# ElementsProject/lightning

Measured on AMD Instinct MI355X. Metric: signature verifies/sec (ECDSA+Schnorr mix), higher is better.
Workload: dtype u32 (256-bit modular integer); 1 GPU; configs[1]+configs[2]: 1000000 ECDSA (65-byte keys, 65536 distinct) + 1000000 BIP-340 Schnorr per GPU per step, 90% valid / 10% invalid, inputs resident in HBM; parallelism=shard-by-row x1, RCCL all-gather of verdicts, key_table_cache=off (tables rebuilt every call)

## Files before the change

### include/lightning_amd.h

```cpp
#ifndef LIGHTNING_AMD_H
#define LIGHTNING_AMD_H
#include <stddef.h>
#include <stdint.h>

#ifdef __cplusplus
extern "C" {
#endif

typedef struct lamd_ctx lamd_ctx;

enum {
	LAMD_OK = 0,
	LAMD_ERR_NO_DEVICE = -1,
	LAMD_ERR_HIP = -2,
	LAMD_ERR_ARG = -3,
	LAMD_ERR_NOMEM = -4,
	LAMD_ERR_STATE = -5
};

int lamd_init(lamd_ctx **ctx, int device);
void lamd_shutdown(lamd_ctx *ctx);
const char *lamd_last_error(const lamd_ctx *ctx);
const char *lamd_version(void);

// ... 117 lines not shown
	uint64_t dropped_deleted, dropped_verdict, dropped_dependency, dropped_bookkeeping;
	uint64_t out_len;
	double stage_ms[3];
} lamd_store_repair_summary;
int lamd_gossip_store_repair(lamd_ctx *ctx, const uint8_t *store, size_t len, const void *d_store, const uint8_t *uuid32, size_t cap,
			     uint64_t *rec_off, int8_t *verdict, uint64_t *new_off, uint8_t *reason, size_t *n_records, uint8_t *out,
			     void *d_out, size_t out_cap, lamd_store_summary *summary, lamd_store_repair_summary *repair);

typedef struct {
	uint64_t now;
	uint32_t future_slack;
	uint32_t prune_interval;
} lamd_store_latest_policy;
typedef struct {
	uint64_t kept;
	uint64_t dropped_deleted, dropped_verdict, dropped_dependency, dropped_bookkeeping,
		 dropped_superseded, dropped_timestamp, dropped_stale;
	uint64_t out_len;
	double stage_ms[3];
} lamd_store_latest_summary;
int lamd_gossip_store_repair_latest(lamd_ctx *ctx, const uint8_t *store, size_t len, const void *d_store, const uint8_t *uuid32,
				    const lamd_store_latest_policy *policy, size_t cap, uint64_t *rec_off, int8_t *verdict, uint64_t *new_off,
				    uint8_t *reason, size_t *n_records, uint8_t *out, void *d_out, size_t out_cap,
				    lamd_store_summary *summary, lamd_store_latest_summary *latest);

int lamd_queue_ecdsa(lamd_ctx *ctx, const uint8_t hash32[32], const uint8_t sig64[64],
		     const uint8_t *pubkey, size_t publen);
int lamd_queue_schnorr(lamd_ctx *ctx, const uint8_t msg32[32], const uint8_t xonly32[32],
		       const uint8_t sig64[64]);
int lamd_queue_ecdsa_batch(lamd_ctx *ctx, size_t n, const uint8_t *hash32, const uint8_t *sig64, const uint8_t *pubkey,
			   size_t publen, size_t pubstride);
int lamd_queue_schnorr_batch(lamd_ctx *ctx, size_t n, const uint8_t *msg32, const uint8_t *xonly32, const uint8_t *sig64);
int lamd_queue_reserve(lamd_ctx *ctx, size_t n, size_t keylen, uint8_t **hash32, uint8_t **sig64, uint8_t **key);
int lamd_queue_ecdsa_batch_inplace(lamd_ctx *ctx, size_t n, const uint8_t *hash32, const uint8_t *sig64, const uint8_t *pubkey, size_t publen);
int lamd_queue_schnorr_batch_inplace(lamd_ctx *ctx, size_t n, const uint8_t *msg32, const uint8_t *xonly32, const uint8_t *sig64);
int lamd_host_register(lamd_ctx *ctx, void *p, size_t bytes);
int lamd_host_unregister(lamd_ctx *ctx, void *p);
int lamd_device_numa_node(int device);
int lamd_flush(lamd_ctx *ctx);
int lamd_poll(lamd_ctx *ctx, uint8_t *ok, size_t cap, size_t *n);
int lamd_wait(lamd_ctx *ctx, uint8_t *ok, size_t cap, size_t *n);

typedef struct lamd_multi lamd_multi;
int lamd_multi_init(lamd_multi **m, const int *devices, int n_devices);
void lamd_multi_shutdown(lamd_multi *m);
const char *lamd_multi_last_error(const lamd_multi *m);
int lamd_multi_devices(const lamd_multi *m);
lamd_ctx *lamd_multi_ctx(lamd_multi *m, int i);
int lamd_multi_verify_ecdsa_batch(lamd_multi *m, size_t n, const uint8_t *hash32, const uint8_t *sig64, const uint8_t *pub, size_t publen,
				  size_t pubstride, size_t group_rows, uint8_t *ok);
int lamd_multi_verify_schnorr_batch(lamd_multi *m, size_t n, const uint8_t *msg32, const uint8_t *xonly32, const uint8_t *sig64, size_t group_rows,
				    uint8_t *ok);
int lamd_multi_sigcheck_gossip_batch(lamd_multi *m, size_t n, const uint8_t *msgs, const uint64_t *off, const uint8_t *node_ids33, int8_t *verdict);
int lamd_shard_bounds(size_t n_groups, const uint32_t *group_rows, int n_shards, size_t *bounds_groups, size_t *bounds_rows);



typedef struct {
	int device;
	int compute_units;
	char arch[64];
	size_t gtable_bytes;
	double last_kernel_ms[4];
	size_t last_unique_keys;
	size_t last_hot_rows;
	int last_keyed;
	int last_mode;
	int lanes;
	size_t last_cache_hits;
	size_t last_cold_rows;
	size_t last_new_tables;
	size_t last_suspect_rows;
	int cache_enabled;
	size_t cache_entries, cache_capacity;
	size_t cache_resets;
	double keyed_ecmult_ms_sum[2];
	size_t keyed_ecmult_launches[2];
	int hw_queues_env;
	int queue_sets;
	size_t last_flush_inplace_rows;
} lamd_info;
int lamd_get_info(lamd_ctx *ctx, lamd_info *info);
int lamd_get_lane_info(lamd_ctx *ctx, int lane, lamd_info *info);
int lamd_set_timing(lamd_ctx *ctx, int enable);
int lamd_cache_clear(lamd_ctx *ctx);
int lamd_set_ecmult_chain(lamd_ctx *ctx, int enable);
int lamd_set_chunk_rows(lamd_ctx *ctx, size_t rows);

#ifdef __cplusplus
}
#endif
#endif
```

### lightning_amd/_build.py

```python
import hashlib
import os
import subprocess

PKG = os.path.dirname(os.path.abspath(__file__))
ROOT = os.path.dirname(PKG)
CSRC = os.path.join(PKG, "csrc")
OBJDIR = os.path.join(PKG, "build")
LIB = os.path.join(PKG, "liblightning_amd.so")
INC = os.path.join(ROOT, "include")
_H = lambda *names: [os.path.join(CSRC, f) for f in names]
_I = lambda *names: [os.path.join(INC, f) for f in names]

HIPFLAGS = ["--offload-arch=gfx950", "-O3", "-std=c++17", "-fPIC", "-pthread", "-Wno-unknown-pragmas", "-mllvm", "-amdgpu-codegenprepare-mul24=false"]
EXTRA = os.environ.get("LAMD_BUILD_FLAGS", "").split()

ENGINE_TUS = [
    ("lamd_engine.hip", _H("verify_core.h", "group.h", "fe.h", "fe_asm.inc", "fuzz.h", "scalar.h", "sha256.h", "lamd_common.h", "bolt12.h", "host_ranges.h", "key_column.h", "store_audit.h", "store_repair.h", "store_latest.h") +
     _I("lightning_amd.h", "lightning_amd_debug.h"), HIPFLAGS + EXTRA),
    ("lamd_multi.cpp", _H("numa_cpus.h") + _I("lightning_amd.h", "lightning_amd_debug.h"), ["-O2", "-std=c++17", "-fPIC", "-pthread", "-Wall"]),
]
SOURCES = sorted({os.path.join(CSRC, tu[0]) for tu in ENGINE_TUS} | {h for tu in ENGINE_TUS for h in tu[1]})

TESTGEN = os.path.join(PKG, "liblightning_amd_testgen.so")
TESTGEN_SOURCES = _H("lamd_testgen.hip", "verify_core.h", "group.h", "fe.h", "fe_asm.inc", "scalar.h", "sha256.h", "lamd_common.h") + _I("lightning_amd_testgen.h")

SHIM = os.path.join(PKG, "liblightning_amd_cln.so")
SHIM_CPP = _H("cln_shim.cpp", "gossip_ingest.cpp")
SHIM_SOURCES = SHIM_CPP + _I("cln_shim.h", "lightning_amd_gossipd.h", "lightning_amd.h") + _H("verify_core.h")


def _digest(files, extra=()):
    h = hashlib.sha256()
    for f in files:
        h.update(os.path.basename(f).encode() + b"\0")
        with open(f, "rb") as fh:
            h.update(fh.read())
    for e in extra:
        h.update(str(e).encode() + b"\0")
    return h.hexdigest()


def _fresh(artefact, digest):
    try:
        return os.path.exists(artefact) and open(artefact + ".stamp").read().strip() == digest
    except OSError:
        return False


def _stamp(artefact, digest):
    with open(artefact + ".stamp", "w") as f:
        f.write(digest + "\n")


def _hipcc():
    return os.environ.get("HIPCC", "/opt/rocm/bin/hipcc")


def _engine_digests():
    return [(src, _digest([os.path.join(CSRC, src)] + deps, flags), flags) for src, deps, flags in ENGINE_TUS]


def is_stale():
    tus = _engine_digests()
    return not _fresh(LIB, _digest([], [d for _, d, _ in tus]))


def build_shim(force=False):
    digest = _digest(SHIM_SOURCES, ["shim-v2"])
    if not force and _fresh(SHIM, digest) and os.path.exists(LIB):
        return SHIM
    cxx = os.environ.get("CXX", "g++")
    subprocess.check_call([cxx, "-O2", "-std=c++17", "-fPIC", "-shared", "-pthread", "-Wall", "-Wno-unknown-pragmas", "-Wno-unused-function", "-o", SHIM + ".tmp"] + SHIM_CPP +
                          ["-L" + PKG, "-llightning_amd", "-Wl,-rpath,$ORIGIN"])
    os.replace(SHIM + ".tmp", SHIM)
    _stamp(SHIM, digest)
    return SHIM


def build_testgen(force=False):
    digest = _digest(TESTGEN_SOURCES, HIPFLAGS)
    if not force and _fresh(TESTGEN, digest) and os.path.exists(LIB):
        return TESTGEN
    subprocess.check_call([_hipcc()] + [f for f in HIPFLAGS if f != "-pthread"] + ["-shared", "-o", TESTGEN + ".tmp", os.path.join(CSRC, "lamd_testgen.hip"),
                           "-L" + PKG, "-llightning_amd", "-Wl,-rpath,$ORIGIN"])
    os.replace(TESTGEN + ".tmp", TESTGEN)
    _stamp(TESTGEN, digest)
    return TESTGEN


SERVED = os.path.join(PKG, "lamd_served")
CLIENT = os.path.join(PKG, "liblightning_amd_client.so")
SHIM_CLIENT = os.path.join(PKG, "liblightning_amd_cln_client.so")
SERVED_SOURCES = _H("lamd_served.cpp", "served_common.h", "numa_cpus.h") + _I("lightning_amd_served.h", "lightning_amd.h")
CLIENT_SOURCES = _H("lamd_client.cpp", "served_common.h") + _I("lightning_amd_served.h", "lightning_amd.h")


def build_served(force=False):
    cxx = os.environ.get("CXX", "g++")
    flags = ["-O2", "-std=c++17", "-fPIC", "-pthread", "-Wall", "-Wno-unknown-pragmas", "-Wno-unused-function"]
    d = _digest(SERVED_SOURCES, ["served-v1"])
# ... 49 lines not shown
```

### lightning_amd/_ffi.py

```python
import ctypes
import os

from . import _build

c_u8p = ctypes.c_void_p
c_sz = ctypes.c_size_t


class LamdTxTemplate(ctypes.Structure):
    _fields_ = [("version", ctypes.c_uint32), ("locktime", ctypes.c_uint32), ("inputs40", ctypes.c_void_p), ("n_inputs", ctypes.c_uint32),
                ("input_num", ctypes.c_uint32), ("amount_sat", ctypes.c_uint64), ("outputs", ctypes.c_void_p), ("outputs_len", ctypes.c_uint64),
                ("n_outputs", ctypes.c_uint32), ("script", ctypes.c_void_p), ("script_len", ctypes.c_uint64)]


class LamdInfo(ctypes.Structure):
    _fields_ = [("device", ctypes.c_int), ("compute_units", ctypes.c_int), ("arch", ctypes.c_char * 64),
                ("gtable_bytes", ctypes.c_size_t), ("last_kernel_ms", ctypes.c_double * 4), ("last_unique_keys", ctypes.c_size_t),
                ("last_hot_rows", ctypes.c_size_t), ("last_keyed", ctypes.c_int), ("last_mode", ctypes.c_int), ("lanes", ctypes.c_int),
                ("last_cache_hits", ctypes.c_size_t), ("last_cold_rows", ctypes.c_size_t), ("last_new_tables", ctypes.c_size_t),
                ("last_suspect_rows", ctypes.c_size_t), ("cache_enabled", ctypes.c_int), ("cache_entries", ctypes.c_size_t),
                ("cache_capacity", ctypes.c_size_t), ("cache_resets", ctypes.c_size_t),
                ("keyed_ecmult_ms_sum", ctypes.c_double * 2), ("keyed_ecmult_launches", ctypes.c_size_t * 2), ("hw_queues_env", ctypes.c_int), ("queue_sets", ctypes.c_int),
                ("last_flush_inplace_rows", ctypes.c_size_t)]


class LamdStoreSummary(ctypes.Structure):
    _fields_ = [("version", ctypes.c_int), ("end_reason", ctypes.c_int), ("clean", ctypes.c_int), ("records", ctypes.c_uint64), ("live", ctypes.c_uint64),
                ("deleted", ctypes.c_uint64), ("end_offset", ctypes.c_uint64), ("ok", ctypes.c_uint64), ("skipped_deleted", ctypes.c_uint64),
                ("bad_checksum", ctypes.c_uint64), ("unknown_type", ctypes.c_uint64), ("malformed", ctypes.c_uint64), ("redundant", ctypes.c_uint64),
                ("no_channel", ctypes.c_uint64), ("bad_signature", ctypes.c_uint64 * 4), ("signatures", ctypes.c_uint64), ("stage_ms", ctypes.c_double * 5)]


class LamdStoreRepairSummary(ctypes.Structure):
    _fields_ = [("kept", ctypes.c_uint64), ("dropped_deleted", ctypes.c_uint64), ("dropped_verdict", ctypes.c_uint64), ("dropped_dependency", ctypes.c_uint64),
                ("dropped_bookkeeping", ctypes.c_uint64), ("out_len", ctypes.c_uint64), ("stage_ms", ctypes.c_double * 3)]


class LamdStoreLatestPolicy(ctypes.Structure):
    _fields_ = [("now", ctypes.c_uint64), ("future_slack", ctypes.c_uint32), ("prune_interval", ctypes.c_uint32)]


class LamdStoreLatestSummary(ctypes.Structure):
    _fields_ = [("kept", ctypes.c_uint64), ("dropped_deleted", ctypes.c_uint64), ("dropped_verdict", ctypes.c_uint64), ("dropped_dependency", ctypes.c_uint64),
                ("dropped_bookkeeping", ctypes.c_uint64), ("dropped_superseded", ctypes.c_uint64), ("dropped_timestamp", ctypes.c_uint64),
                ("dropped_stale", ctypes.c_uint64), ("out_len", ctypes.c_uint64), ("stage_ms", ctypes.c_double * 3)]


SYMBOLS = {
    "lamd_init": (ctypes.c_int, [ctypes.POINTER(ctypes.c_void_p), ctypes.c_int]),
    "lamd_shutdown": (None, [ctypes.c_void_p]),
    "lamd_last_error": (ctypes.c_char_p, [ctypes.c_void_p]),
    "lamd_version": (ctypes.c_char_p, []),
    "lamd_verify_ecdsa_batch": (ctypes.c_int, [ctypes.c_void_p, c_sz, c_u8p, c_u8p, c_u8p, c_sz, c_sz, c_u8p]),
    "lamd_verify_schnorr_batch": (ctypes.c_int, [ctypes.c_void_p, c_sz, c_u8p, c_u8p, c_u8p, c_u8p]),
    "lamd_verify_ecdsa_batch_device": (ctypes.c_int, [ctypes.c_void_p, c_sz, c_u8p, c_u8p, c_u8p, c_sz, c_sz, c_u8p]),
    "lamd_verify_schnorr_batch_device": (ctypes.c_int, [ctypes.c_void_p, c_sz, c_u8p, c_u8p, c_u8p, c_u8p]),
    "lamd_stream": (ctypes.c_void_p, [ctypes.c_void_p]),
    "lamd_synchronize": (ctypes.c_int, [ctypes.c_void_p]),
    "lamd_check_signed_hash": (ctypes.c_int, [ctypes.c_void_p, c_u8p, c_u8p, c_u8p, c_sz]),
    "lamd_check_signed_hash_nodeid": (ctypes.c_int, [ctypes.c_void_p, c_u8p, c_u8p, c_u8p]),
    "lamd_check_schnorr_sig": (ctypes.c_int, [ctypes.c_void_p, c_u8p, c_u8p, c_u8p]),
    "lamd_check_tx_sig_batch": (ctypes.c_int, [ctypes.c_void_p, c_sz, c_u8p, c_u8p, c_u8p, c_u8p, c_u8p, c_u8p, c_sz, c_sz, c_u8p]),
    "lamd_check_tx_sig_tx_batch": (ctypes.c_int, [ctypes.c_void_p, c_sz] + [c_u8p] * 15 + [c_sz, c_sz, c_u8p]),
    "lamd_check_commitment_signed": (ctypes.c_int, [ctypes.c_void_p, ctypes.c_void_p, c_u8p, c_u8p, ctypes.c_uint8, c_sz, ctypes.c_void_p, c_u8p, c_u8p, c_u8p,
                                                    ctypes.POINTER(ctypes.c_int64), c_u8p]),
    "lamd_bolt12_check_signature_batch": (ctypes.c_int, [ctypes.c_void_p, c_sz, c_u8p, c_u8p, ctypes.c_char_p, ctypes.c_char_p, c_u8p, c_sz, c_u8p, c_u8p]),
    "lamd_bolt12_merkle_batch": (ctypes.c_int, [ctypes.c_void_p, c_sz, c_u8p, c_u8p, ctypes.c_char_p, ctypes.c_char_p, c_u8p, c_u8p, c_u8p]),
    "lamd_ecdsa_recover_batch": (ctypes.c_int, [ctypes.c_void_p, c_sz, c_u8p, c_u8p, c_u8p, c_u8p, c_u8p]),
    "lamd_ecdsa_recover_batch_device": (ctypes.c_int, [ctypes.c_void_p, c_sz, c_u8p, c_u8p, c_u8p, c_u8p, c_u8p]),
    "lamd_grind_htlc_tx_fee": (ctypes.c_int, [ctypes.c_void_p, c_u8p, c_sz, c_u8p, c_sz, ctypes.c_uint64, ctypes.c_uint64, ctypes.c_uint32,
                                              ctypes.c_uint32, c_u8p, ctypes.c_uint8, ctypes.c_int, c_u8p, ctypes.POINTER(ctypes.c_uint32),
                                              ctypes.POINTER(ctypes.c_uint64)]),
    "lamd_pubkey_parse_batch": (ctypes.c_int, [ctypes.c_void_p, c_sz, c_u8p, c_sz, c_sz, c_u8p, c_u8p]),
    "lamd_sigcheck_gossip_batch": (ctypes.c_int, [ctypes.c_void_p, c_sz, c_u8p, c_u8p, c_u8p, c_u8p]),
    "lamd_queue_ecdsa": (ctypes.c_int, [ctypes.c_void_p, c_u8p, c_u8p, c_u8p, c_sz]),
    "lamd_queue_schnorr": (ctypes.c_int, [ctypes.c_void_p, c_u8p, c_u8p, c_u8p]),
    "lamd_queue_ecdsa_batch": (ctypes.c_int, [ctypes.c_void_p, c_sz, c_u8p, c_u8p, c_u8p, c_sz, c_sz]),
    "lamd_queue_schnorr_batch": (ctypes.c_int, [ctypes.c_void_p, c_sz, c_u8p, c_u8p, c_u8p]),
    "lamd_flush": (ctypes.c_int, [ctypes.c_void_p]),
    "lamd_poll": (ctypes.c_int, [ctypes.c_void_p, c_u8p, c_sz, ctypes.POINTER(c_sz)]),
    "lamd_wait": (ctypes.c_int, [ctypes.c_void_p, c_u8p, c_sz, ctypes.POINTER(c_sz)]),
    "lamd_sigcheck_gossip_batch_device": (ctypes.c_int, [ctypes.c_void_p, c_sz, c_u8p, c_u8p, c_u8p, c_u8p, c_sz, c_u8p]),
    "lamd_sigcheck_gossip_spans_device": (ctypes.c_int, [ctypes.c_void_p, c_sz, c_u8p, c_u8p, c_u8p, c_u8p, c_u8p, c_sz, c_u8p]),
    "lamd_gossip_store_frame": (ctypes.c_int, [c_u8p, c_sz, c_sz, c_u8p, ctypes.POINTER(c_sz), ctypes.POINTER(LamdStoreSummary)]),
    "lamd_gossip_store_audit": (ctypes.c_int, [ctypes.c_void_p, c_u8p, c_sz, ctypes.c_void_p, c_sz, c_u8p, c_u8p, ctypes.POINTER(c_sz), ctypes.POINTER(LamdStoreSummary)]),
    "lamd_gossip_store_repair": (ctypes.c_int, [ctypes.c_void_p, c_u8p, c_sz, ctypes.c_void_p, c_u8p, c_sz, c_u8p, c_u8p, c_u8p, c_u8p, ctypes.POINTER(c_sz), c_u8p,
                                                ctypes.c_void_p, c_sz, ctypes.POINTER(LamdStoreSummary), ctypes.POINTER(LamdStoreRepairSummary)]),
    "lamd_gossip_store_repair_latest": (ctypes.c_int, [ctypes.c_void_p, c_u8p, c_sz, ctypes.c_void_p, c_u8p, ctypes.POINTER(LamdStoreLatestPolicy), c_sz, c_u8p, c_u8p,
                                                       c_u8p, c_u8p, ctypes.POINTER(c_sz), c_u8p, ctypes.c_void_p, c_sz, ctypes.POINTER(LamdStoreSummary),
                                                       ctypes.POINTER(LamdStoreLatestSummary)]),
    "lamd_selftest": (ctypes.c_int, [ctypes.c_void_p, c_u8p, c_u8p, c_u8p, ctypes.c_char_p, c_sz]),
    "lamd_chain_debug": (ctypes.c_int, [ctypes.c_void_p, ctypes.c_int, ctypes.c_char_p, c_sz]),
    "lamd_inv_debug": (ctypes.c_int, [ctypes.c_void_p, ctypes.c_char_p, c_sz]),
    "lamd_x2_debug": (ctypes.c_int, [ctypes.c_void_p, ctypes.c_char_p, c_sz]),
    "lamd_debug_read": (ctypes.c_int, [ctypes.c_void_p, ctypes.c_int, c_sz, c_sz, c_u8p]),
    "lamd_debug_mul32_peak": (ctypes.c_int, [ctypes.c_void_p, ctypes.c_int, ctypes.c_double, ctypes.c_int] + [ctypes.POINTER(ctypes.c_double)] * 3),
    "lamd_debug_gtable": (ctypes.c_void_p, [ctypes.c_void_p]),
    "lamd_fuzz_field": (ctypes.c_int, [ctypes.c_void_p, c_sz, ctypes.c_int, ctypes.c_uint64, ctypes.POINTER(ctypes.c_uint64), ctypes.c_char_p, c_sz]),
    "lamd_get_info": (ctypes.c_int, [ctypes.c_void_p, ctypes.POINTER(LamdInfo)]),
    "lamd_set_timing": (ctypes.c_int, [ctypes.c_void_p, ctypes.c_int]),
    "lamd_set_ecmult_chain": (ctypes.c_int, [ctypes.c_void_p, ctypes.c_int]),
    "lamd_set_chunk_rows": (ctypes.c_int, [ctypes.c_void_p, c_sz]),
    "lamd_cache_clear": (ctypes.c_int, [ctypes.c_void_p]),
    "lamd_get_lane_info": (ctypes.c_int, [ctypes.c_void_p, ctypes.c_int, ctypes.POINTER(LamdInfo)]),
    "lamd_stream_wait_results": (ctypes.c_int, [ctypes.c_void_p, ctypes.c_void_p]),
    "lamd_wait_stream": (ctypes.c_int, [ctypes.c_void_p, ctypes.c_void_p]),
    "lamd_wait_event": (ctypes.c_int, [ctypes.c_void_p, ctypes.c_void_p]),
    "lamd_queue_reserve": (ctypes.c_int, [ctypes.c_void_p, c_sz, c_sz] + [ctypes.POINTER(ctypes.c_void_p)] * 3),
    "lamd_queue_ecdsa_batch_inplace": (ctypes.c_int, [ctypes.c_void_p, c_sz, c_u8p, c_u8p, c_u8p, c_sz]),
    "lamd_queue_schnorr_batch_inplace": (ctypes.c_int, [ctypes.c_void_p, c_sz, c_u8p, c_u8p, c_u8p]),
    "lamd_host_register": (ctypes.c_int, [ctypes.c_void_p, ctypes.c_void_p, c_sz]),
    "lamd_host_unregister": (ctypes.c_int, [ctypes.c_void_p, ctypes.c_void_p]),
    "lamd_device_numa_node": (ctypes.c_int, [ctypes.c_int]),
    "lamd_results_mark": (ctypes.c_int, [ctypes.c_void_p, ctypes.c_int]),
    "lamd_results_mark_last": (ctypes.c_int, [ctypes.c_void_p, ctypes.c_int]),
    "lamd_stream_wait_mark": (ctypes.c_int, [ctypes.c_void_p, ctypes.c_int, ctypes.c_void_p]),
    "lamd_multi_init": (ctypes.c_int, [ctypes.POINTER(ctypes.c_void_p), ctypes.POINTER(ctypes.c_int), ctypes.c_int]),
    "lamd_multi_init_backend": (ctypes.c_int, [ctypes.POINTER(ctypes.c_void_p), ctypes.POINTER(ctypes.c_int), ctypes.c_int, ctypes.c_void_p]),
    "lamd_multi_shutdown": (None, [ctypes.c_void_p]),
    "lamd_multi_last_error": (ctypes.c_char_p, [ctypes.c_void_p]),
    "lamd_multi_devices": (ctypes.c_int, [ctypes.c_void_p]),
    "lamd_multi_ctx": (ctypes.c_void_p, [ctypes.c_void_p, ctypes.c_int]),
    "lamd_multi_verify_ecdsa_batch": (ctypes.c_int, [ctypes.c_void_p, c_sz, c_u8p, c_u8p, c_u8p, c_sz, c_sz, c_sz, c_u8p]),
    "lamd_multi_verify_schnorr_batch": (ctypes.c_int, [ctypes.c_void_p, c_sz, c_u8p, c_u8p, c_u8p, c_sz, c_u8p]),
    "lamd_multi_sigcheck_gossip_batch": (ctypes.c_int, [ctypes.c_void_p, c_sz, c_u8p, c_u8p, c_u8p, c_u8p]),
    "lamd_shard_bounds": (ctypes.c_int, [c_sz, c_u8p, ctypes.c_int, c_u8p, c_u8p]),
}

TESTGEN_SYMBOLS = {
    "lamd_gen_ecdsa_device": (ctypes.c_int, [ctypes.c_void_p, c_sz, ctypes.c_uint64, c_sz, c_sz, c_sz, c_u8p, c_u8p, c_u8p]),
    "lamd_gen_schnorr_device": (ctypes.c_int, [ctypes.c_void_p, c_sz, ctypes.c_uint64, c_sz, c_sz, c_u8p, c_u8p, c_u8p]),
    "lamd_gen_gossip_device": (ctypes.c_int, [ctypes.c_void_p, c_sz, c_sz, ctypes.c_uint64, c_sz, c_u8p, c_u8p]),
}

_lib = None
_testgen = None


def load(build_if_needed=True):
    global _lib
    if _lib is None:
        alt = os.environ.get("LAMD_LIB_PATH")
        if alt:
            L = ctypes.CDLL(alt)
            for name, (res, args) in SYMBOLS.items():
                f = getattr(L, name)
                f.restype = res
                f.argtypes = args
            _lib = L
            return _lib
        if build_if_needed and os.path.exists("/opt/rocm/bin/hipcc"):
            _build.build()
        if not os.path.exists(_build.LIB):
            raise RuntimeError("liblightning_amd.so is not built (run `python -c 'import __graft_entry__ as g; g.build()'`); "
                               "lightning_amd has no CPU fallback")
        L = ctypes.CDLL(_build.LIB)
        for name, (res, args) in SYMBOLS.items():
            f = getattr(L, name)
            f.restype = res
            f.argtypes = args
        _lib = L
    return _lib


def load_testgen():
    global _testgen
    if _testgen is None:
        load()
        alt = os.environ.get("LAMD_TESTGEN_LIB_PATH")
        path = alt if alt else (_build.build_testgen() if os.path.exists("/opt/rocm/bin/hipcc") else _build.TESTGEN)
        L = ctypes.CDLL(path)
        for name, (res, args) in TESTGEN_SYMBOLS.items():
            f = getattr(L, name)
            f.restype = res
            f.argtypes = args
        _testgen = L
    return _testgen
```

### lightning_amd/csrc/lamd_engine.hip

```cpp
#include <hip/hip_runtime.h>
#include <type_traits>
#include <stdio.h>
#include <stdlib.h>
#include <string.h>

#include <map>
#include <mutex>
#include <random>
#include <string>
#include <atomic>
#include <thread>
#include <vector>

#include "../../include/lightning_amd.h"
#include "../../include/lightning_amd_debug.h"
#include "verify_core.h"
#include "fuzz.h"
#include "host_ranges.h"
#include "key_column.h"
#include "store_audit.h"
#include "store_repair.h"
#include "store_latest.h"

using namespace lamd;

constexpr int MAX_LANES = 8;

__device__ u32 g_prio;
#ifndef LAMD_PRIO_DEFAULT
#define LAMD_PRIO_DEFAULT 13
#endif
#define LAMD_PRIO(bit)                                     \
  do {                                                     \
    if (g_prio & (bit)) __builtin_amdgcn_s_setprio(3);     \
  } while (0)


__global__ void __launch_bounds__(256) k_gtable_build(u32 *__restrict__ gtable, const u32 *__restrict__ bases) {
  const size_t idx = (size_t)blockIdx.x * blockDim.x + threadIdx.x;
  if (idx >= GTABLE_ENTRIES) return;
  const u32 w = (u32)(idx >> GTABLE_WINDOW_BITS), d = (u32)(idx & ((1u << GTABLE_WINDOW_BITS) - 1u));
  u32 out[GT_ENTRY_WORDS];
  if (d == 0) {
#pragma unroll
    for (int i = 0; i < GT_ENTRY_WORDS; i++) out[i] = 0;
  } else {
    u32 base[16];
#pragma unroll
    for (int i = 0; i < 16; i++) base[i] = bases[w * 16 + i];
    gtable_compute_entry(out, base, d);
  }
  uint2 *dst = reinterpret_cast<uint2 *>(gtable + idx * GT_ENTRY_WORDS);
#pragma unroll
  for (int i = 0; i < GT_ENTRY_WORDS / 2; i++) dst[i] = make_uint2(out[2 * i], out[2 * i + 1]);
}

__global__ void __launch_bounds__(256) k_ecdsa_prep(size_t n, const u8 *__restrict__ hash32, const u8 *__restrict__ sig64,
                                                    prep_rec *__restrict__ recs) {
  LAMD_PRIO(4);
  const size_t tid = (size_t)blockIdx.x * blockDim.x + threadIdx.x;
  const size_t T = (size_t)gridDim.x * blockDim.x;
  ecdsa_prep_thread(tid, T, n, hash32, sig64, recs);
}

__global__ void __launch_bounds__(256) k_schnorr_prep(size_t n, const u8 *__restrict__ msg32, const u8 *__restrict__ pk32,
                                                      const u8 *__restrict__ sig64, prep_rec *__restrict__ recs) {
  LAMD_PRIO(4);
  const size_t i = (size_t)blockIdx.x * blockDim.x + threadIdx.x;
  if (i >= n) return;
  schnorr_prep_one(msg32 + 32 * i, pk32 + 32 * i, sig64 + 64 * i, &recs[i]);
}

constexpr int FIN_WORDS = 32;

__global__ void __launch_bounds__(256) k_keys(size_t n, const u8 *__restrict__ pub, int publen, size_t stride,
                                              const u32 *__restrict__ idx, u32 *__restrict__ qwords, u8 *__restrict__ keyok,
                                              const u32 *__restrict__ count) {
  const size_t i = (size_t)blockIdx.x * blockDim.x + threadIdx.x;
  if (i >= n || (count && i >= *count)) return;
  const size_t row = idx ? idx[i] : i;
  u32 qx[8], qy[8];
  const bool ok = parse_pubkey(pub + stride * row, publen, qx, qy);
  uint4 *dst = reinterpret_cast<uint4 *>(qwords + i * 16);
  dst[0] = make_uint4(qx[0], qx[1], qx[2], qx[3]);
  dst[1] = make_uint4(qx[4], qx[5], qx[6], qx[7]);
  dst[2] = make_uint4(qy[0], qy[1], qy[2], qy[3]);
  dst[3] = make_uint4(qy[4], qy[5], qy[6], qy[7]);
  keyok[i] = ok;
}

__device__ __forceinline__ u32 wave_alloc(u32 *counter, bool pred, u32 weight = 0, u32 *wsum = nullptr);
__global__ void __launch_bounds__(256) k_keys_cold(size_t n, const u8 *__restrict__ pub, int publen, size_t stride, const u32 *__restrict__ idx,
                                                   const u32 *__restrict__ count, u32 *__restrict__ counter_ok, u32 *__restrict__ idx_ok,
                                                   u32 *__restrict__ qwords, u8 *__restrict__ keyok_row, u8 *__restrict__ out) {
  LAMD_PRIO(2);
  const size_t i = (size_t)blockIdx.x * blockDim.x + threadIdx.x;
  const bool live = i < n && i < *count;
  const size_t row = live ? idx[i] : 0;
  u32 qx[8], qy[8];
  const bool ok = live && parse_pubkey(pub + stride * row, publen, qx, qy);
  const u32 pos = wave_alloc(counter_ok, ok, 0, nullptr);
  if (!live) return;
// ... 1332 lines not shown
    const bool last = gridDim.x == 1u || __hip_atomic_fetch_add(A.done, 1u, __ATOMIC_ACQ_REL, __HIP_MEMORY_SCOPE_AGENT) == gridDim.x - 1u;
    if (last) {
      if (gridDim.x != 1u) __hip_atomic_store(A.done, 0u, __ATOMIC_RELAXED, __HIP_MEMORY_SCOPE_AGENT);
      __hip_atomic_store(A.flag, A.ticket, __ATOMIC_RELEASE, __HIP_MEMORY_SCOPE_SYSTEM);
    }
  }
}

__global__ void __launch_bounds__(256) k_schnorr_final_fin(size_t n, u32 *__restrict__ fin, u8 *__restrict__ out) {
  LAMD_PRIO(16);
  const size_t tid = (size_t)blockIdx.x * blockDim.x + threadIdx.x;
  const size_t T = (size_t)gridDim.x * blockDim.x;
  schnorr_final_thread(tid, T, n, fin, out, FIN_WORDS);
}


static constexpr size_t CHUNK_DEFAULT = (size_t)1 << 22;

struct devbuf {
  void *p = nullptr;
  size_t cap = 0;
  template <class T> T *as() const { return static_cast<T *>(p); }
};

enum { Q_ECDSA33 = 0, Q_ECDSA65 = 1, Q_SCHNORR = 2, Q_KINDS = 3 };
#ifndef LAMD_QUEUE_SETS
#define LAMD_QUEUE_SETS 9
#endif
constexpr int QUEUE_SETS = LAMD_QUEUE_SETS;

struct shared_gtable { std::mutex mu; u32 *p = nullptr; int refs = 0; };
static std::mutex g_gtable_mu;
static std::map<int, shared_gtable> g_gtables;
static shared_gtable &gtable_slot(int device) {
  std::lock_guard<std::mutex> lk(g_gtable_mu);
  return g_gtables[device];
}

struct lamd_ctx {
  int device = 0;
  int gtable_device = -1;
  hipStream_t stream = nullptr;
  hipDeviceProp_t prop;
  u32 *gtable = nullptr;
  std::string err;
  devbuf recs, qwords, keyok, slots, vbuf;
  devbuf row_ent, kd_table, kd_rep, kd_uid, kd_uniq, kd_count, kd_newent, plan, kt_fin;
  struct shape_ws { devbuf row, ent, slot, qwords, keyok, scratch; } hk[2];
  devbuf list7, list10, listcold, listcold_ok;
  u8 *h_small = nullptr;
  u8 *h_tmpl = nullptr;
  size_t h_tmpl_cap = 0;
  devbuf small_done;
  std::vector<u64> small_missed;
  u32 prio_mask = LAMD_PRIO_DEFAULT;
  unsigned spin_us = 2000;
  std::vector<u64> learn_fps;
  devbuf learn_dev;
  bool force_learn = false;
  u32 small_ticket = 0;
  bool small_kernel = true;
  u32 *h_plan = nullptr;
  struct key_cache {
    bool shared = false;
    u32 cap_ent = 0, cap7 = 0, cap10 = 0, index_mask = 0;
    devbuf ents, index, pool7, pool10, counters;
  } cache_store;
  key_cache *cache = nullptr;
  lamd_ctx *root = nullptr;
  int lane_id = 0;
  u32 call_seq = 0;
  u32 pub_seq[MAX_LANES + 1] = {};
  hipEvent_t ev_pub[MAX_LANES + 1] = {};
  u32 vis_seq[MAX_LANES + 1] = {};
  bool pub_pending[MAX_LANES + 1] = {};
  int cache_mode = 1;
  size_t cache_keys = (size_t)1 << 20, cache_keys10 = (size_t)1 << 16;
  u32 cache_hwm[3] = {0, 0, 0};
  u32 cache_resets = 0;
  size_t last_hits = 0, last_cold = 0, last_l7 = 0, last_l10 = 0;
  devbuf keyok_row;
  hipStream_t stream2 = nullptr;
  hipStream_t stream3 = nullptr;
  hipEvent_t ev_fork = nullptr, ev_prep = nullptr, ev_cold = nullptr, ev_keys = nullptr, ev_sigs = nullptr;
  bool sigs_pending = false;
  hipEvent_t ev_sigs_wait = nullptr;
  static constexpr int MAX_COPY_STREAMS = 4;
  hipStream_t copy_streams[MAX_COPY_STREAMS] = {nullptr, nullptr, nullptr, nullptr};
  int n_copy_streams = 1;
  bool copy_one = true;
  int copy_events = 0;
  unsigned copy_turn = 0;
  bool use_copy_stream = true;
  int keyed_mode = -1;
  size_t keyed_min_rows = 8192;
  bool early_cold = true;
  bool fused_front = true;
  bool kc_tree = false;
  bool small_fused = true;
  bool last_small_fused = false;
  size_t last_small_n = 0;
  double keyed_min_uses = 6.0;
  double keyed_dense_uses = 48.0;
  int keyed_teeth = 0;
  int last_mode = 0;
  size_t last_n = 0;
  bool last_keyed_call = false;
  devbuf in_a, in_b, in_c, out;
  devbuf g_msgs, g_off, g_ids, g_rowbase, g_hash, g_sig, g_pub, g_malformed, g_ok, g_verdict;
  devbuf st_img, st_host, st_ids, st_tab, st_out;
  hipEvent_t ev_store[6] = {};
  devbuf st_rep, st_pack;
  hipEvent_t ev_rep[4] = {};
  bool timing = false;
  bool ev_recorded = false;
  int ecmult_waves = 3;
  bool pairs = false;
  bool group_rows = true;
  devbuf g_cnt, g_base, g_rank, g_touched, g_list7, g_list10;
  devbuf pairs_ws;
  size_t prep_batch = 16;
  size_t prep_min_threads = 0;
  u64 hash_seed = 0x243F6A8885A308D3ULL;
  size_t chunk = CHUNK_DEFAULT;
  hipEvent_t ev[5] = {nullptr, nullptr, nullptr, nullptr, nullptr};
  double last_ms[4] = {0, 0, 0, 0};
  static const int MARK_SLOTS = 16;
  hipEvent_t ev_mark[MARK_SLOTS][MAX_LANES + 1] = {};
  bool mark_set[MARK_SLOTS] = {};
  int mark_only[MARK_SLOTS] = {-1, -1, -1, -1, -1, -1, -1, -1, -1, -1, -1, -1, -1, -1, -1, -1};
  static const int KEV = 64;
  hipEvent_t kev[KEV][2] = {};
  int kev_mode[KEV] = {};
  int kev_n = 0;
  double keyed_ms_sum[2] = {0, 0};
  size_t keyed_launches[2] = {0, 0};
  struct queue {
    u8 *h_blk = nullptr;
    u8 *h_a = nullptr, *h_b = nullptr, *h_c = nullptr, *h_ok = nullptr;
    size_t cap = 0, n = 0;
    static size_t key_bytes_padded(size_t cap, size_t keybytes) { return (cap * keybytes + 63) & ~(size_t)63; }
    static size_t blk_bytes(size_t cap, size_t keybytes) { return key_bytes_padded(cap, keybytes) + cap * 96; }
    struct span { size_t row0; u32 ticket0; size_t count; };
    std::vector<span> tickets;
    struct foreign_span { size_t row0, count; const u8 *a, *b, *c; };
    std::vector<foreign_span> foreign;
    devbuf d_blk, d_ok;
    hipEvent_t ev_keys = nullptr, ev_sigs = nullptr, ev_all = nullptr;
    bool small_flush = false;
  };
  struct queue_set {
    queue q[Q_KINDS];
    hipEvent_t done = nullptr;
    size_t rows = 0;
  } qs[QUEUE_SETS];
  int q_open = 0;
  int q_fifo[QUEUE_SETS] = {0};
  int q_inflight = 0;
  size_t last_flush_inplace_rows = 0;
  lamd_ctx *lane[MAX_LANES] = {};
  int nlanes = 0;
  lamd_ctx *peer = nullptr;
  lamd_ctx *last_lane = nullptr;
  lamd_ctx *last_chunk_lane = nullptr;
  bool is_lane = false;
  int next_lane = 0;
  hipEvent_t ev_lane = nullptr, ev_join = nullptr;
  hipEvent_t ev_ecm[MAX_LANES + 1] = {};
  int ecm_last = -1;
  int ecm_chain = 0;
  size_t ecm_chain_min = 65536;
  u32 ecm_tail = 131072;
  hipStream_t stream_lo = nullptr;
  hipEvent_t ev_lo_go = nullptr, ev_lo_done = nullptr;
};

#define HIPCHK(ctx, call)                                                                           \
  do {                                                                                              \
    hipError_t e_ = (call);                                                                         \
    if (e_ != hipSuccess) {                                                                         \
      (ctx)->err = std::string(#call) + ": " + hipGetErrorString(e_);                               \
      return LAMD_ERR_HIP;                                                                          \
    }                                                                                               \
  } while (0)

static int ensure(lamd_ctx *ctx, devbuf *b, size_t bytes) {
  if (bytes <= b->cap) return LAMD_OK;
  if (b->p) {
    HIPCHK(ctx, hipDeviceSynchronize());
    HIPCHK(ctx, hipFree(b->p));
  }
  b->p = nullptr;
  b->cap = 0;
  size_t want = bytes + bytes / 4 + 4096;
  if (hipMalloc(&b->p, want) != hipSuccess) {
    want = bytes;
    hipError_t e = hipMalloc(&b->p, want);
    if (e != hipSuccess) {
      ctx->err = std::string("hipMalloc: ") + hipGetErrorString(e);
      return LAMD_ERR_NOMEM;
    }
  }
  b->cap = want;
  return LAMD_OK;
}
static void release(devbuf *b) {
  if (b->p) (void)hipFree(b->p);
  b->p = nullptr;
  b->cap = 0;
}


static inline unsigned blocks_for(size_t n) { return (unsigned)((n + 255) / 256); }
static unsigned careful_grid(const lamd_ctx *ctx, size_t n) {
  const bool flood = ctx->h_plan && ((volatile const u32 *)ctx->h_plan)[P_SUSPECT] > 4096u;
  return flood || blocks_for(n) < 64u ? blocks_for(n) : 64u;
}

static unsigned keyed_grid(size_t n) { return (unsigned)((n + KEYED_THREADS - 1) / KEYED_THREADS); }

static int hw_queues_from_env(void) {
  const char *v = getenv("GPU_MAX_HW_QUEUES");
  return v && *v ? atoi(v) : 0;
}

extern "C" const char *lamd_version(void) { return "lightning_amd 0.1 (gfx950)"; }

extern "C" const char *lamd_last_error(const lamd_ctx *ctx) { return ctx ? ctx->err.c_str() : "no context"; }

static int init_known_answers(lamd_ctx *ctx);
static int cache_alloc(lamd_ctx *owner, lamd_ctx::key_cache *kc, size_t keys7, size_t keys10, bool shared);
static int cache_reset(lamd_ctx *root);
static int cache_maybe_reset(lamd_ctx *root);

static int create_streams(lamd_ctx *ctx) {
  HIPCHK(ctx, hipStreamCreateWithFlags(&ctx->stream, hipStreamNonBlocking));
  HIPCHK(ctx, hipStreamCreateWithFlags(&ctx->stream2, hipStreamNonBlocking));
  if (!getenv("LAMD_MERGE_SIDE") || atoi(getenv("LAMD_MERGE_SIDE")) != 0) ctx->stream3 = ctx->stream2;
  else HIPCHK(ctx, hipStreamCreateWithFlags(&ctx->stream3, hipStreamNonBlocking));
  HIPCHK(ctx, hipEventCreateWithFlags(&ctx->ev_cold, hipEventDisableTiming));
  HIPCHK(ctx, hipEventCreateWithFlags(&ctx->ev_keys, hipEventDisableTiming));
  HIPCHK(ctx, hipEventCreateWithFlags(&ctx->ev_sigs, hipEventDisableTiming));
  HIPCHK(ctx, hipEventCreateWithFlags(&ctx->ev_fork, hipEventDisableTiming));
  HIPCHK(ctx, hipEventCreateWithFlags(&ctx->ev_prep, hipEventDisableTiming));
  HIPCHK(ctx, hipHostMalloc((void **)&ctx->h_plan, (P_WORDS + C_WORDS) * 4, hipHostMallocDefault));
  memset(ctx->h_plan, 0, (P_WORDS + C_WORDS) * 4);
  if (!ctx->is_lane)
    for (auto &e : ctx->ev_pub) HIPCHK(ctx, hipEventCreateWithFlags(&e, hipEventDisableTiming));
  HIPCHK(ctx, hipEventCreateWithFlags(&ctx->ev_lane, hipEventDisableTiming));
  HIPCHK(ctx, hipEventCreateWithFlags(&ctx->ev_join, hipEventDisableTiming));
  if (getenv("LAMD_ECMULT_CHAIN") && atoi(getenv("LAMD_ECMULT_CHAIN")) == 2) {
    int lo = 0, hi = 0;
    HIPCHK(ctx, hipDeviceGetStreamPriorityRange(&lo, &hi));
    HIPCHK(ctx, hipStreamCreateWithPriority(&ctx->stream_lo, hipStreamNonBlocking, lo));
    HIPCHK(ctx, hipEventCreateWithFlags(&ctx->ev_lo_go, hipEventDisableTiming));
    HIPCHK(ctx, hipEventCreateWithFlags(&ctx->ev_lo_done, hipEventDisableTiming));
  }
  for (auto &e : ctx->ev) HIPCHK(ctx, hipEventCreate(&e));
  if (!ctx->is_lane) {
    for (auto &qs : ctx->qs) {
      HIPCHK(ctx, hipEventCreateWithFlags(&qs.done, hipEventDisableTiming));
      for (auto &q : qs.q)
        for (hipEvent_t *e : {&q.ev_keys, &q.ev_sigs, &q.ev_all}) HIPCHK(ctx, hipEventCreateWithFlags(e, hipEventDisableTiming));
    }
    if (const char *w = getenv("LAMD_COPY_ONE")) ctx->copy_one = atoi(w) != 0;
    if (const char *w = getenv("LAMD_COPY_EVENTS")) ctx->copy_events = atoi(w) < 0 ? 0 : atoi(w) > 3 ? 3 : atoi(w);
    if (const char *w = getenv("LAMD_COPY_STREAMS")) ctx->n_copy_streams = atoi(w) < 1 ? 1 : atoi(w) > lamd_ctx::MAX_COPY_STREAMS ? lamd_ctx::MAX_COPY_STREAMS : atoi(w);
    for (auto &e : ctx->ev_ecm) HIPCHK(ctx, hipEventCreateWithFlags(&e, hipEventDisableTiming));
    if (const char *w = getenv("LAMD_ECMULT_CHAIN")) ctx->ecm_chain = atoi(w);
    if (const char *w = getenv("LAMD_ECMULT_TAIL")) ctx->ecm_tail = (u32)atol(w);
    if (const char *w = getenv("LAMD_COPY_STREAM")) ctx->use_copy_stream = atoi(w) != 0;
  }
  return LAMD_OK;
}
static int make_lanes(lamd_ctx *root, int count) {
  for (int i = 0; i < count; i++) {
    lamd_ctx *L = new (std::nothrow) lamd_ctx();
    if (!L) return LAMD_ERR_NOMEM;
    root->lane[i] = L;
    L->is_lane = true;
    L->root = root;
    L->lane_id = i + 1;
    L->cache_mode = root->cache_mode;
    L->device = root->device;
    L->prop = root->prop;
    L->gtable = root->gtable;
    L->ecmult_waves = root->ecmult_waves;
    L->pairs = root->pairs;
    L->group_rows = root->group_rows;
    L->prep_batch = root->prep_batch;
    L->prep_min_threads = root->prep_min_threads;
    L->hash_seed = root->hash_seed;
    L->chunk = root->chunk;
    L->keyed_mode = root->keyed_mode;
    L->keyed_min_rows = root->keyed_min_rows;
    L->small_fused = root->small_fused;
    L->fused_front = root->fused_front;
    L->early_cold = root->early_cold;
    L->keyed_min_uses = root->keyed_min_uses;
    L->keyed_dense_uses = root->keyed_dense_uses;
    L->keyed_teeth = root->keyed_teeth;
    const int rc = create_streams(L);
    if (rc != LAMD_OK) { root->err = L->err; return rc; }
  }
  root->nlanes = count;
  for (int i = 0; i < count; i++) root->lane[i]->peer = root->lane[(i + 1) % count];
  return LAMD_OK;
}
static int pick_lane(lamd_ctx *root, lamd_ctx **out) {
  *out = root;
  const int rcc = cache_maybe_reset(root);
  if (rcc != LAMD_OK) return rcc;
  if (!root->lane[0]) return LAMD_OK;
  lamd_ctx *L = root->lane[root->next_lane];
  root->next_lane = (root->next_lane + 1) % root->nlanes;
  root->last_lane = L;
  L->timing = root->timing;
  HIPCHK(root, hipEventRecord(root->ev_lane, root->stream));
  HIPCHK(root, hipStreamWaitEvent(L->stream, root->ev_lane, 0));
  *out = L;
  return LAMD_OK;
}

extern "C" int lamd_init(lamd_ctx **out, int device) {
  if (!out) return LAMD_ERR_ARG;
  *out = nullptr;
  int count = 0;
  if (hipGetDeviceCount(&count) != hipSuccess || count <= 0) return LAMD_ERR_NO_DEVICE;
  if (device < 0 || device >= count) return LAMD_ERR_ARG;
  lamd_ctx *ctx = new (std::nothrow) lamd_ctx();
  if (!ctx) return LAMD_ERR_NOMEM;
  ctx->device = device;
  *out = ctx;
  HIPCHK(ctx, hipSetDevice(device));
  HIPCHK(ctx, hipGetDeviceProperties(&ctx->prop, device));
  if (strncmp(ctx->prop.gcnArchName, "gfx950", 6) != 0) {
    ctx->err = std::string("unsupported architecture ") + ctx->prop.gcnArchName + " (built for gfx950 only)";
    return LAMD_ERR_NO_DEVICE;
  }
  if (const char *w = getenv("LAMD_ECMULT_WAVES")) ctx->ecmult_waves = atoi(w);
  if (const char *w = getenv("LAMD_PAIRS")) ctx->pairs = atoi(w) != 0;
  if (const char *w = getenv("LAMD_GROUP")) ctx->group_rows = atoi(w) != 0;
  if (const char *w = getenv("LAMD_SPIN_US")) ctx->spin_us = (unsigned)atoi(w);
  if (const char *w = getenv("LAMD_PRIO")) ctx->prio_mask = (u32)atoi(w);
  if (const char *w = getenv("LAMD_FUSED_FRONT")) ctx->fused_front = atoi(w) != 0;
  if (const char *w = getenv("LAMD_EARLY_COLD")) ctx->early_cold = atoi(w) != 0;
  if (const char *w = getenv("LAMD_KC_TREE")) ctx->kc_tree = atoi(w) != 0;
  if (const char *w = getenv("LAMD_PREP_BATCH")) ctx->prep_batch = atoi(w) < 1 ? 1 : (size_t)atoi(w);
  if (const char *w = getenv("LAMD_PREP_MIN_THREADS")) ctx->prep_min_threads = atol(w) < 0 ? 0 : (size_t)atol(w);
  {
    std::random_device rd;
    ctx->hash_seed = ((u64)rd() << 32) ^ (u64)rd() ^ 0x243F6A8885A308D3ULL;
  }
  if (const char *w = getenv("LAMD_CHUNK_ROWS")) ctx->chunk = (size_t)atoll(w) < 4 ? 4 : (size_t)atoll(w);
  if (const char *w = getenv("LAMD_KEYED")) ctx->keyed_mode = atoi(w);
  if (const char *w = getenv("LAMD_KEYED_MIN_USES")) ctx->keyed_min_uses = atof(w);
  if (const char *w = getenv("LAMD_KEYED_DENSE_USES")) ctx->keyed_dense_uses = atof(w);
  if (const char *w = getenv("LAMD_KEYED_TEETH")) ctx->keyed_teeth = atoi(w) == 7 ? 7 : (atoi(w) == 10 ? 10 : 0);
  if (const char *w = getenv("LAMD_KEYED_MIN_ROWS")) ctx->keyed_min_rows = (size_t)atoll(w);
  if (const char *w = getenv("LAMD_SMALL_FUSED")) ctx->small_fused = atoi(w) != 0;
  if (const char *w = getenv("LAMD_CACHE")) ctx->cache_mode = atoi(w) != 0;
  if (const char *w = getenv("LAMD_SMALL_KERNEL")) ctx->small_kernel = atoi(w) != 0;
  if (const char *w = getenv("LAMD_CACHE_KEYS")) ctx->cache_keys = (size_t)atoll(w) < 64 ? 64 : (size_t)atoll(w);
  if (const char *w = getenv("LAMD_CACHE_KEYS10")) ctx->cache_keys10 = (size_t)atoll(w) < 16 ? 16 : (size_t)atoll(w);
  int rc = create_streams(ctx);
  if (rc != LAMD_OK) return rc;
  std::vector<u32> bases(GTABLE_WINDOWS * 16);
  {
    const u32 gx[8] = LAMD_GX, gy[8] = LAMD_GY;
    u32 cur[16];
    memcpy(cur, gx, 32);
    memcpy(cur + 8, gy, 32);
    for (int w = 0; w < GTABLE_WINDOWS; w++) {
      memcpy(&bases[w * 16], cur, 64);
      gej b = gej_from_ge(ge_from_words(cur, cur + 8));
      for (int i = 0; i < GTABLE_WINDOW_BITS; i++) b = gej_double(b);
      const fe zi = fe_inv(fe_norm_weak(b.z));
      const fe zi2 = fe_sqr(zi);
      fe_to_words(cur, fe_normalize(fe_mul(b.x, zi2)));
      fe_to_words(cur + 8, fe_normalize(fe_mul(b.y, fe_mul(zi2, zi))));
    }
  }
  HIPCHK(ctx, hipMemcpyToSymbol(HIP_SYMBOL(g_prio), &ctx->prio_mask, sizeof(u32)));
  {
    shared_gtable &sg = gtable_slot(device);
    std::lock_guard<std::mutex> lk(sg.mu);
    if (sg.refs == 0) {
      u32 *d_bases = nullptr;
      const char *what = "hipMalloc (window bases)";
      hipError_t e = hipMalloc(&d_bases, bases.size() * 4);
      if (e == hipSuccess) { what = "hipMemcpy (window bases)"; e = hipMemcpy(d_bases, bases.data(), bases.size() * 4, hipMemcpyHostToDevice); }
      if (e == hipSuccess) { what = "hipMalloc (static G table, 11 GiB)"; e = hipMalloc(&sg.p, GTABLE_BYTES); }
      if (e == hipSuccess) {
        what = "k_gtable_build";
        hipLaunchKernelGGL(k_gtable_build, dim3(blocks_for(GTABLE_ENTRIES)), dim3(256), 0, ctx->stream, sg.p, d_bases);
        e = hipGetLastError();
        if (e == hipSuccess) e = hipStreamSynchronize(ctx->stream);
      }
      if (d_bases) (void)hipFree(d_bases);
      if (e != hipSuccess) {
        if (sg.p) (void)hipFree(sg.p);
        sg.p = nullptr;
        (void)hipGetLastError();
        ctx->err = std::string(what) + ": " + hipGetErrorString(e);
        return e == hipErrorOutOfMemory ? LAMD_ERR_NOMEM : LAMD_ERR_HIP;
      }
    }
    sg.refs++;
    ctx->gtable = sg.p;
    ctx->gtable_device = device;
  }
  if (ctx->cache_mode) {
    if ((rc = cache_alloc(ctx, &ctx->cache_store, ctx->cache_keys, ctx->cache_keys10, true)) != LAMD_OK) return rc;
    if ((rc = cache_reset(ctx)) != LAMD_OK) return rc;
    ctx->cache_resets = 0;
  }
  const char *lanes = getenv("LAMD_LANES");
  const int nl = lanes ? atoi(lanes) : 6;
  if (nl > 1) {
    rc = make_lanes(ctx, nl > MAX_LANES ? MAX_LANES : nl);
    if (rc != LAMD_OK) return rc;
  }
  return init_known_answers(ctx);
}

extern "C" void lamd_shutdown(lamd_ctx *ctx) {
  if (!ctx) return;
  (void)hipSetDevice(ctx->device);
  for (auto &L : ctx->lane) {
    if (L) lamd_shutdown(L);
    L = nullptr;
  }
  for (hipStream_t cs : ctx->copy_streams)
    if (cs) (void)hipStreamSynchronize(cs);
  if (ctx->stream) (void)hipStreamSynchronize(ctx->stream);
  for (devbuf *b : {&ctx->row_ent, &ctx->kd_table, &ctx->kd_rep, &ctx->kd_uid, &ctx->kd_uniq, &ctx->kd_count, &ctx->kd_newent, &ctx->plan,
                    &ctx->kt_fin, &ctx->list7,
                    &ctx->list10, &ctx->listcold, &ctx->listcold_ok, &ctx->keyok_row, &ctx->pairs_ws, &ctx->g_cnt, &ctx->g_base, &ctx->g_rank, &ctx->g_touched, &ctx->g_list7, &ctx->g_list10, &ctx->cache_store.ents, &ctx->cache_store.index, &ctx->cache_store.pool7,
                    &ctx->cache_store.pool10, &ctx->cache_store.counters})
    release(b);
  for (auto &w : ctx->hk)
    for (devbuf *b : {&w.row, &w.ent, &w.slot, &w.qwords, &w.keyok, &w.scratch}) release(b);
  for (auto &e : ctx->ev_pub)
    if (e) (void)hipEventDestroy(e);
  if (ctx->stream2) { (void)hipStreamSynchronize(ctx->stream2); (void)hipStreamDestroy(ctx->stream2); }
  if (ctx->stream3 && ctx->stream3 != ctx->stream2) { (void)hipStreamSynchronize(ctx->stream3); (void)hipStreamDestroy(ctx->stream3); }
  if (ctx->ev_cold) (void)hipEventDestroy(ctx->ev_cold);
  if (ctx->ev_keys) (void)hipEventDestroy(ctx->ev_keys);
  if (ctx->ev_sigs) (void)hipEventDestroy(ctx->ev_sigs);
  if (ctx->ev_fork) (void)hipEventDestroy(ctx->ev_fork);
  if (ctx->ev_prep) (void)hipEventDestroy(ctx->ev_prep);
  for (devbuf *b : {&ctx->small_done, &ctx->recs, &ctx->qwords, &ctx->keyok, &ctx->slots, &ctx->vbuf, &ctx->in_a, &ctx->in_b, &ctx->in_c, &ctx->out,
                    &ctx->g_msgs, &ctx->g_off, &ctx->g_ids, &ctx->g_rowbase, &ctx->g_hash, &ctx->g_sig, &ctx->g_pub,
                    &ctx->g_malformed, &ctx->g_ok, &ctx->g_verdict, &ctx->st_img, &ctx->st_host, &ctx->st_ids, &ctx->st_tab, &ctx->st_out, &ctx->st_rep,
                    &ctx->st_pack})
    release(b);
  for (auto &e : ctx->ev_store)
    if (e) (void)hipEventDestroy(e);
  for (auto &e : ctx->ev_rep)
    if (e) (void)hipEventDestroy(e);
  for (auto &qs : ctx->qs) {
    for (auto &q : qs.q) {
      q.h_a = q.h_b = q.h_c = nullptr;
      for (u8 **h : {&q.h_blk, &q.h_ok})
        if (*h) (void)hipHostFree(*h);
      for (devbuf *b : {&q.d_blk, &q.d_ok}) release(b);
      for (hipEvent_t e : {q.ev_keys, q.ev_sigs, q.ev_all})
        if (e) (void)hipEventDestroy(e);
    }
    if (qs.done) (void)hipEventDestroy(qs.done);
  }
  for (hipStream_t cs : ctx->copy_streams)
    if (cs) (void)hipStreamDestroy(cs);
  for (auto &e : ctx->ev_ecm)
    if (e) (void)hipEventDestroy(e);
  if (ctx->gtable && !ctx->is_lane) {
    shared_gtable &sg = gtable_slot(ctx->gtable_device);
    std::lock_guard<std::mutex> lk(sg.mu);
    if (sg.refs > 0 && --sg.refs == 0) {
      (void)hipFree(sg.p);
      sg.p = nullptr;
    }
    ctx->gtable = nullptr;
  }
  if (ctx->h_plan) (void)hipHostFree(ctx->h_plan);
  if (ctx->h_small) (void)hipHostFree(ctx->h_small);
  if (ctx->h_tmpl) (void)hipHostFree(ctx->h_tmpl);
  if (ctx->stream_lo) { (void)hipStreamSynchronize(ctx->stream_lo); (void)hipStreamDestroy(ctx->stream_lo); }
  for (hipEvent_t e : {ctx->ev_lo_go, ctx->ev_lo_done})
    if (e) (void)hipEventDestroy(e);
  if (ctx->ev_lane) (void)hipEventDestroy(ctx->ev_lane);
  if (ctx->ev_join) (void)hipEventDestroy(ctx->ev_join);
  for (auto &e : ctx->ev)
    if (e) (void)hipEventDestroy(e);
  for (auto &pair : ctx->kev)
    for (auto &e : pair)
      if (e) (void)hipEventDestroy(e);
  for (auto &slot : ctx->ev_mark)
    for (auto &e : slot)
      if (e) (void)hipEventDestroy(e);
  if (ctx->stream) (void)hipStreamDestroy(ctx->stream);
  delete ctx;
}

extern "C" void *lamd_stream(lamd_ctx *ctx) { return ctx ? (void *)ctx->stream : nullptr; }

extern "C" int lamd_synchronize(lamd_ctx *ctx) {
  if (!ctx) return LAMD_ERR_ARG;
  for (lamd_ctx *L : ctx->lane) {
    if (!L) continue;
    const int rc = lamd_synchronize(L);
    if (rc != LAMD_OK) { ctx->err = L->err; return rc; }
  }
  HIPCHK(ctx, hipStreamSynchronize(ctx->stream));
  if (ctx->timing && ctx->ev_recorded) {
    for (int i = 0; i < 4; i++) {
      float ms = 0;
      if (hipEventElapsedTime(&ms, ctx->ev[i], ctx->ev[i + 1]) == hipSuccess) ctx->last_ms[i] = ms;
    }
    (void)hipGetLastError();
  }
  for (int i = 0; i < ctx->kev_n; i++) {
    float ms = 0;
    if (hipEventElapsedTime(&ms, ctx->kev[i][0], ctx->kev[i][1]) == hipSuccess) {
      ctx->keyed_ms_sum[ctx->kev_mode[i]] += ms;
      ctx->keyed_launches[ctx->kev_mode[i]]++;
    }
  }
  (void)hipGetLastError();
  ctx->kev_n = 0;
  return LAMD_OK;
}

extern "C" int lamd_stream_wait_results(lamd_ctx *ctx, void *stream) {
  if (!ctx) return LAMD_ERR_ARG;
  for (int i = 0; i <= MAX_LANES; i++) {
    lamd_ctx *L = i < MAX_LANES ? ctx->lane[i] : ctx;
    if (!L) continue;
    HIPCHK(ctx, hipEventRecord(L->ev_join, L->stream));
    HIPCHK(ctx, hipStreamWaitEvent((hipStream_t)stream, L->ev_join, 0));
  }
  return LAMD_OK;
}
extern "C" int lamd_wait_event(lamd_ctx *ctx, void *event) {
  if (!ctx || !event) return LAMD_ERR_ARG;
  HIPCHK(ctx, hipStreamWaitEvent(ctx->stream, (hipEvent_t)event, 0));
  return LAMD_OK;
}
extern "C" int lamd_results_mark(lamd_ctx *ctx, int slot) {
  if (!ctx || slot < 0 || slot >= lamd_ctx::MARK_SLOTS) return LAMD_ERR_ARG;
  HIPCHK(ctx, hipSetDevice(ctx->device));
  for (int i = 0; i <= MAX_LANES; i++) {
    lamd_ctx *L = i < MAX_LANES ? ctx->lane[i] : ctx;
    hipEvent_t &e = ctx->ev_mark[slot][i];
    if (!L) continue;
    if (!e) HIPCHK(ctx, hipEventCreateWithFlags(&e, hipEventDisableTiming));
    HIPCHK(ctx, hipEventRecord(e, L->stream));
  }
  ctx->mark_set[slot] = true;
  ctx->mark_only[slot] = -1;
  return LAMD_OK;
}
extern "C" int lamd_results_mark_last(lamd_ctx *ctx, int slot) {
  if (!ctx || slot < 0 || slot >= lamd_ctx::MARK_SLOTS) return LAMD_ERR_ARG;
  HIPCHK(ctx, hipSetDevice(ctx->device));
  int idx = MAX_LANES;
  lamd_ctx *L = ctx;
  for (int i = 0; i < MAX_LANES; i++)
    if (ctx->lane[i] && ctx->lane[i] == ctx->last_lane) { idx = i; L = ctx->lane[i]; }
  hipEvent_t &e = ctx->ev_mark[slot][idx];
  if (!e) HIPCHK(ctx, hipEventCreateWithFlags(&e, hipEventDisableTiming));
  HIPCHK(ctx, hipEventRecord(e, L->stream));
  ctx->mark_set[slot] = true;
  ctx->mark_only[slot] = idx;
  return LAMD_OK;
}
extern "C" int lamd_stream_wait_mark(lamd_ctx *ctx, int slot, void *stream) {
  if (!ctx || slot < 0 || slot >= lamd_ctx::MARK_SLOTS) return LAMD_ERR_ARG;
  if (!ctx->mark_set[slot]) {
    ctx->err = "lamd_stream_wait_mark: slot was never marked";
    return LAMD_ERR_STATE;
  }
  if (ctx->mark_only[slot] >= 0) {
    HIPCHK(ctx, hipStreamWaitEvent((hipStream_t)stream, ctx->ev_mark[slot][ctx->mark_only[slot]], 0));
    return LAMD_OK;
  }
  for (int i = 0; i <= MAX_LANES; i++)
    if (ctx->ev_mark[slot][i]) HIPCHK(ctx, hipStreamWaitEvent((hipStream_t)stream, ctx->ev_mark[slot][i], 0));
  return LAMD_OK;
}

extern "C" int lamd_wait_stream(lamd_ctx *ctx, void *stream) {
  if (!ctx) return LAMD_ERR_ARG;
  HIPCHK(ctx, hipEventRecord(ctx->ev_fork, (hipStream_t)stream));
  HIPCHK(ctx, hipStreamWaitEvent(ctx->stream, ctx->ev_fork, 0));
  return LAMD_OK;
}

extern "C" int lamd_set_timing(lamd_ctx *ctx, int enable) {
  if (!ctx) return LAMD_ERR_ARG;
  ctx->timing = enable != 0;
  for (lamd_ctx *L : ctx->lane)
    if (L) L->timing = ctx->timing;
  for (int i = 0; i <= MAX_LANES; i++) {
    lamd_ctx *L = i < MAX_LANES ? ctx->lane[i] : ctx;
    if (!L) continue;
    L->kev_n = 0;
    L->keyed_ms_sum[0] = L->keyed_ms_sum[1] = 0;
    L->keyed_launches[0] = L->keyed_launches[1] = 0;
  }
  return LAMD_OK;
}

extern "C" int lamd_set_chunk_rows(lamd_ctx *ctx, size_t rows) {
  if (!ctx) return LAMD_ERR_ARG;
  const size_t c = rows == 0 ? CHUNK_DEFAULT : rows < 4096 ? 4096 : rows > CHUNK_DEFAULT ? CHUNK_DEFAULT : rows;
  ctx->chunk = c;
  for (lamd_ctx *L : ctx->lane)
    if (L) L->chunk = c;
  return LAMD_OK;
}

extern "C" int lamd_set_ecmult_chain(lamd_ctx *ctx, int enable) {
  if (!ctx) return LAMD_ERR_ARG;
  ctx->ecm_chain = enable != 0;
  ctx->ecm_last = -1;
  return LAMD_OK;
}

static int get_info_of(lamd_ctx *ctx, lamd_info *info);
extern "C" int lamd_get_info(lamd_ctx *ctx, lamd_info *info) {
  if (!ctx || !info) return LAMD_ERR_ARG;
  const int rc = get_info_of(ctx->last_lane ? ctx->last_lane : ctx, info);
  info->lanes = ctx->nlanes ? ctx->nlanes : 1;
  return rc;
}
extern "C" int lamd_get_lane_info(lamd_ctx *ctx, int lane, lamd_info *info) {
  if (!ctx || !info || lane < 0 || lane >= (ctx->nlanes ? ctx->nlanes : 1)) return LAMD_ERR_ARG;
  const int rc = get_info_of(ctx->lane[lane] ? ctx->lane[lane] : ctx, info);
  info->lanes = ctx->nlanes ? ctx->nlanes : 1;
  return rc;
}
static int get_info_of(lamd_ctx *ctx, lamd_info *info) {
  lamd_ctx *root = ctx->root ? ctx->root : ctx;
  const lamd_ctx *self = ctx;
  if (ctx->last_chunk_lane) ctx = ctx->last_chunk_lane;
  memset(info, 0, sizeof(*info));
  info->device = ctx->device;
  info->compute_units = ctx->prop.multiProcessorCount;
  strncpy(info->arch, ctx->prop.gcnArchName, sizeof(info->arch) - 1);
  info->gtable_bytes = GTABLE_BYTES;
  info->hw_queues_env = hw_queues_from_env();
  info->queue_sets = QUEUE_SETS;
  info->last_flush_inplace_rows = root->last_flush_inplace_rows;
  for (int i = 0; i < 4; i++) info->last_kernel_ms[i] = ctx->last_ms[i];
  for (int i = 0; i < 2; i++) {
    info->keyed_ecmult_ms_sum[i] = self->keyed_ms_sum[i];
    info->keyed_ecmult_launches[i] = self->keyed_launches[i];
  }
  info->last_mode = ctx->last_mode;
  if (ctx->last_keyed_call && ctx->h_plan) {
    const volatile u32 *h = ctx->h_plan;
    info->last_unique_keys = h[P_UNIQ];
    info->last_hot_rows = (size_t)h[P_L7] + h[P_L10];
    info->last_keyed = h[P_L10] ? 10 : (h[P_L7] ? 7 : 0);
    info->last_cache_hits = h[P_HITS];
    info->last_cold_rows = h[P_COLD];
    info->last_new_tables = (size_t)h[P_HK7] + h[P_HK10];
    info->last_suspect_rows = h[P_SUSPECT];
  }
  info->cache_enabled = root->cache_mode != 0 && root->cache_store.shared;
  info->cache_entries = root->cache_hwm[0];
  info->cache_capacity = root->cache_store.cap_ent;
  info->cache_resets = root->cache_resets;
  return LAMD_OK;
}

static void launch_prep(lamd_ctx *ctx, hipStream_t st, int mode, size_t n, const u8 *d_a, const u8 *d_sig, const u8 *d_key, prep_rec *recs) {
  if (mode == MODE_ECDSA) {
    size_t threads = (n + ctx->prep_batch - 1) / ctx->prep_batch;
    const size_t min_threads = ctx->prep_min_threads ? ctx->prep_min_threads : (size_t)ctx->prop.multiProcessorCount * 256;
    if (threads < min_threads) threads = n < min_threads ? n : min_threads;
    hipLaunchKernelGGL(k_ecdsa_prep, dim3(blocks_for(threads)), dim3(256), 0, st, n, d_a, d_sig, recs);
  } else {
    hipLaunchKernelGGL(k_schnorr_prep, dim3(blocks_for(n)), dim3(256), 0, st, n, d_a, d_key, d_sig, recs);
  }
}
static size_t final_threads(lamd_ctx *ctx, size_t n) {
  size_t threads = (n + 15) / 16;
  const size_t min_threads = (size_t)ctx->prop.multiProcessorCount * 256;
  if (threads < min_threads) threads = n < min_threads ? n : min_threads;
  return threads;
}

static int launch_direct(lamd_ctx *ctx, hipStream_t st, int mode, size_t m, const u32 *idx, const u32 *count, const prep_rec *recs, const u8 *d_sig,
                         const u8 *d_key, int keylen, size_t keystride, u32 *fin, u8 *keyok_row, u8 *d_ok, bool time_it, u32 *plan = nullptr) {
  int rc;
  if ((rc = ensure(ctx, &ctx->qwords, m * 64)) != LAMD_OK) return rc;
  if ((rc = ensure(ctx, &ctx->keyok, m)) != LAMD_OK) return rc;
  if ((rc = ensure(ctx, &ctx->slots, m * SLOT_WORDS * 4)) != LAMD_OK) return rc;
  auto kern = ctx->ecmult_waves == 2 ? k_ecmult<2> : ctx->ecmult_waves == 4 ? k_ecmult<4> : k_ecmult<3>;
  if (idx && count && plan) {
    if ((rc = ensure(ctx, &ctx->listcold_ok, m * 4)) != LAMD_OK) return rc;
    hipLaunchKernelGGL(k_keys_cold, dim3(blocks_for(m)), dim3(256), 0, st, m, d_key, keylen, keystride, idx, count, plan + P_COLDOK,
                       ctx->listcold_ok.as<u32>(), ctx->qwords.as<u32>(), keyok_row, d_ok);
    HIPCHK(ctx, hipStreamWaitEvent(st, ctx->ev_prep, 0));
    hipLaunchKernelGGL(kern, dim3(blocks_for(m)), dim3(256), 0, st, m, recs, ctx->qwords.as<const u32>(), (const u8 *)nullptr, d_sig, mode,
                       (const u32 *)ctx->gtable, ctx->slots.as<u32>(), ctx->listcold_ok.as<const u32>(), fin, keyok_row, d_ok, (const u32 *)(plan + P_COLDOK));
    return LAMD_OK;
// ... 19 lines not shown
    kc->cap7 = (u32)keys7;
    kc->cap10 = (u32)keys10;
    if (shared) {
      size_t m = 1;
      while (m < 2 * ents) m <<= 1;
      if ((rc = ensure(owner, &kc->index, m * 4)) != LAMD_OK) return rc;
      kc->index_mask = (u32)(m - 1);
    }
  }
  return LAMD_OK;
}
static int cache_reset(lamd_ctx *root) {
  lamd_ctx::key_cache *kc = &root->cache_store;
  HIPCHK(root, hipDeviceSynchronize());
  HIPCHK(root, hipMemset(kc->ents.p, 0, (size_t)kc->cap_ent * sizeof(cache_ent)));
  HIPCHK(root, hipMemset(kc->index.p, 0, ((size_t)kc->index_mask + 1) * 4));
  HIPCHK(root, hipMemset(kc->counters.p, 0, C_WORDS * 4));
  for (int l = 0; l <= MAX_LANES; l++) { root->pub_seq[l] = root->vis_seq[l] = 0; root->pub_pending[l] = false; }
  root->call_seq = 0;
  root->cache_hwm[0] = root->cache_hwm[1] = root->cache_hwm[2] = 0;
  for (lamd_ctx *L : root->lane)
    if (L && L->h_plan) memset(L->h_plan, 0, (P_WORDS + C_WORDS) * 4);
  if (root->h_plan) memset(root->h_plan, 0, (P_WORDS + C_WORDS) * 4);
  root->cache_resets++;
  return LAMD_OK;
}
extern "C" int lamd_cache_clear(lamd_ctx *ctx) {
  if (!ctx) return LAMD_ERR_ARG;
  if (ctx->cache_mode == 0 || !ctx->cache_store.shared) return LAMD_OK;
  HIPCHK(ctx, hipSetDevice(ctx->device));
  return cache_reset(ctx);
}


struct chunk_io {
  int mode;
  size_t n;
  const u8 *d_sig, *d_key;
  int keylen;
  size_t keystride;
  u8 *d_ok_caller;
  u8 *keyok_out;
  bool time_it;
  prep_rec *recs;
  u8 *d_ok;
};
struct keyed_lists {
  u32 *plan;
  const u32 *list7, *list10, *row_ent;
  const cache_ent *ents;
  const u32 *pool7, *pool10;
  u32 *fin;
};
template <bool CAREFUL>
static void launch_keyed(lamd_ctx *ctx, hipStream_t st, unsigned grid, const chunk_io &c, const keyed_lists &k, int part = 0, u32 tail = 0) {
  hipLaunchKernelGGL((k_ecmult_keyed<CAREFUL, 3>), dim3(grid), dim3(KEYED_THREADS), 0, st, k.plan, k.list7, k.list10, (const prep_rec *)c.recs, k.row_ent, k.ents,
                     k.pool7, k.pool10, c.d_sig, c.mode, (const u32 *)ctx->gtable, k.fin, c.keyok_out, c.d_ok, part, tail);
}

static cache_vis cache_visibility(lamd_ctx *root, const lamd_ctx *ctx) {
  for (int l = 0; l <= MAX_LANES; l++)
    if (root->pub_pending[l] && hipEventQuery(root->ev_pub[l]) == hipSuccess) {
      root->vis_seq[l] = root->pub_seq[l];
      root->pub_pending[l] = false;
    }
  (void)hipGetLastError();
  cache_vis vis;
  for (int l = 0; l <= MAX_LANES; l++) vis.seq[l] = root->vis_seq[l];
  vis.seq[ctx->lane_id] = root->pub_seq[ctx->lane_id];
  return vis;
}

static int launch_cold(lamd_ctx *ctx, const chunk_io &c, const u32 *listcold, u32 *plan, u32 *fin) {
  HIPCHK(ctx, hipEventRecord(ctx->ev_fork, ctx->stream));
  HIPCHK(ctx, hipStreamWaitEvent(ctx->stream3, ctx->ev_fork, 0));
  const int rc = launch_direct(ctx, ctx->stream3, c.mode, c.n, listcold, plan + P_COLD, c.recs, c.d_sig, c.d_key, c.keylen, c.keystride, fin, c.keyok_out, c.d_ok,
                               false, plan);
  if (rc != LAMD_OK) return rc;
  HIPCHK(ctx, hipEventRecord(ctx->ev_cold, ctx->stream3));
  return LAMD_OK;
}

static int finish_call(lamd_ctx *ctx, const chunk_io &c, u32 *fin, const u32 *plan, const u32 *cc) {
  if (c.time_it) HIPCHK(ctx, hipEventRecord(ctx->ev[3], ctx->stream));
  if (c.mode == MODE_SCHNORR) {
    const unsigned blocks = blocks_for(final_threads(ctx, c.n));
    if (fin) hipLaunchKernelGGL(k_schnorr_final_fin, dim3(blocks), dim3(256), 0, ctx->stream, c.n, fin, c.d_ok);
    else hipLaunchKernelGGL(k_schnorr_final, dim3(blocks), dim3(256), 0, ctx->stream, c.n, ctx->slots.as<u32>(), c.d_ok);
  }
  HIPCHK(ctx, hipMemcpyAsync(c.d_ok_caller, c.d_ok, c.n, hipMemcpyDeviceToDevice, ctx->stream));
  if (plan) HIPCHK(ctx, hipMemcpyAsync(ctx->h_plan, plan, P_WORDS * 4, hipMemcpyDeviceToHost, ctx->stream));
  if (cc) HIPCHK(ctx, hipMemcpyAsync(ctx->h_plan + P_WORDS, cc, C_WORDS * 4, hipMemcpyDeviceToHost, ctx->stream));
  if (c.time_it) {
    HIPCHK(ctx, hipEventRecord(ctx->ev[4], ctx->stream));
    ctx->ev_recorded = true;
  }
  HIPCHK(ctx, hipGetLastError());
  return LAMD_OK;
}

static int chunk_direct(lamd_ctx *ctx, const chunk_io &c) {
  if (c.time_it) HIPCHK(ctx, hipEventRecord(ctx->ev[1], ctx->stream));
  const int rc = launch_direct(ctx, ctx->stream, c.mode, c.n, nullptr, nullptr, c.recs, c.d_sig, c.d_key, c.keylen, c.keystride, nullptr, c.keyok_out, c.d_ok, c.time_it);
  if (rc != LAMD_OK) return rc;
  return finish_call(ctx, c, nullptr, nullptr, nullptr);
}

static int chunk_small_cached(lamd_ctx *ctx, lamd_ctx *root, const chunk_io &c) {
  int rc;
  const size_t n = c.n;
  lamd_ctx::key_cache *kc = &root->cache_store;
  for (devbuf *b : {&ctx->row_ent, &ctx->list7, &ctx->list10, &ctx->listcold})
    if ((rc = ensure(ctx, b, n * 4)) != LAMD_OK) return rc;
  if ((rc = ensure(ctx, &ctx->plan, P_WORDS * 4)) != LAMD_OK) return rc;
  if (c.mode == MODE_SCHNORR && (rc = ensure(ctx, &ctx->kt_fin, n * (size_t)FIN_WORDS * 4)) != LAMD_OK) return rc;
  u32 *plan = ctx->plan.as<u32>();
  const keyed_lists k = {plan, ctx->list7.as<const u32>(), ctx->list10.as<const u32>(), ctx->row_ent.as<const u32>(), kc->ents.as<const cache_ent>(),
                         kc->pool7.as<const u32>(), kc->pool10.as<const u32>(), c.mode == MODE_SCHNORR ? ctx->kt_fin.as<u32>() : nullptr};
  HIPCHK(ctx, hipMemsetAsync(plan, 0, P_WORDS * 4, ctx->stream));
  const cache_vis vis = cache_visibility(root, ctx);
  hipLaunchKernelGGL(k_small_lookup, dim3((unsigned)((n + 63) / 64)), dim3(64), 0, ctx->stream, n, c.d_key, c.keylen, c.keystride, root->hash_seed,
                     kc->index.as<const u32>(), kc->index_mask, k.ents, vis, ctx->row_ent.as<u32>(), plan, ctx->list7.as<u32>(), ctx->list10.as<u32>(),
                     ctx->listcold.as<u32>(), c.keyok_out, c.d_ok);
  if (c.time_it) HIPCHK(ctx, hipEventRecord(ctx->ev[1], ctx->stream));
  if ((rc = launch_cold(ctx, c, ctx->listcold.as<const u32>(), plan, k.fin)) != LAMD_OK) return rc;
  if (c.time_it) HIPCHK(ctx, hipEventRecord(ctx->ev[2], ctx->stream));
  HIPCHK(ctx, hipStreamWaitEvent(ctx->stream, ctx->ev_prep, 0));
  launch_keyed<false>(ctx, ctx->stream, keyed_grid(n), c, k);
  launch_keyed<true>(ctx, ctx->stream, careful_grid(ctx, n), c, k);
  HIPCHK(ctx, hipStreamWaitEvent(ctx->stream, ctx->ev_cold, 0));
  return finish_call(ctx, c, k.fin, plan, nullptr);
}

constexpr u32 NO_TABLES = 0xFFFFFFFFu;
struct front_args {
  lamd_ctx::key_cache *kc;
  bool use_cache;
  size_t m;
  u32 thr[2];
  size_t cap[2];
  u32 seq;
  cache_vis vis;
  learn_filter lf;
  u32 *plan, *cc, *row_ent, *list7, *list10, *listcold, *fin;
};
static kc_shape_args shape_args(const lamd_ctx::shape_ws &w, size_t cap, const devbuf &pool) {
  return {(u32)cap, w.row.as<const u32>(), w.ent.as<const u32>(), w.slot.as<const u32>(), w.qwords.as<u32>(), w.keyok.as<u8>(), w.scratch.as<u32>(), pool.as<u32>()};
}
static int wait_sigs(lamd_ctx *ctx) {
  if (ctx->sigs_pending) {
    HIPCHK(ctx, hipStreamWaitEvent(ctx->stream, ctx->ev_sigs_wait, 0));
    ctx->sigs_pending = false;
  }
  return LAMD_OK;
}
static int launch_cache_lookup(lamd_ctx *ctx, lamd_ctx *root, const chunk_io &c, const front_args &f) {
  const int rc = wait_sigs(ctx);
  if (rc != LAMD_OK) return rc;
  hipLaunchKernelGGL(k_cache_lookup, dim3(blocks_for(c.n)), dim3(256), 0, ctx->stream, c.n, c.d_key, c.keylen, c.keystride, root->hash_seed,
                     f.kc->index.as<const u32>(), f.kc->index_mask, f.kc->ents.as<const cache_ent>(), f.vis, f.row_ent, f.plan, f.list7, f.list10, c.keyok_out, c.d_ok,
                     c.d_sig, c.mode);
  return LAMD_OK;
}
template <bool BYROW>
static void launch_classify(lamd_ctx *ctx, const chunk_io &c, const front_args &f) {
  const cache_caps caps = {f.kc->cap_ent, f.kc->cap7, f.kc->cap10};
  const lamd_ctx::shape_ws &w7 = ctx->hk[0], &w10 = ctx->hk[1];
  hipLaunchKernelGGL((k_dedupe_classify<BYROW>), dim3(blocks_for(c.n)), dim3(256), 0, ctx->stream, c.n, ctx->kd_count.as<const u32>(), ctx->kd_uniq.as<const u32>(),
                     f.thr[0], f.thr[1], f.plan, f.cc, caps, (u32)f.cap[0], (u32)f.cap[1], ctx->kd_newent.as<u32>(), w7.row.as<u32>(), w7.ent.as<u32>(),
                     w7.slot.as<u32>(), w10.row.as<u32>(), w10.ent.as<u32>(), w10.slot.as<u32>(), f.lf);
}
static int mark_published(lamd_ctx *ctx, lamd_ctx *root, const front_args &f) {
  if (f.use_cache) {
    HIPCHK(ctx, hipEventRecord(root->ev_pub[ctx->lane_id], ctx->stream));
    root->pub_seq[ctx->lane_id] = f.seq;
    root->pub_pending[ctx->lane_id] = true;
  }
  return wait_sigs(ctx);
}

static int front_end_fused(lamd_ctx *ctx, lamd_ctx *root, const chunk_io &c, const front_args &f, bool *cold_started) {
  int rc;
  const size_t n = c.n;
  lamd_ctx::key_cache *kc = f.kc;
  {
    const size_t words = f.m > n ? f.m : n;
    const unsigned ib = blocks_for(words / 4 + 1);
    hipLaunchKernelGGL(k_call_init, dim3(ib < 2048u ? ib : 2048u), dim3(256), 0, ctx->stream, f.plan, ctx->kd_table.as<u32>(), f.m, ctx->kd_count.as<u32>(), n,
                       f.use_cache ? (u32 *)nullptr : f.row_ent, f.use_cache ? (u32 *)nullptr : f.cc);
  }
  if (f.use_cache && (rc = launch_cache_lookup(ctx, root, c, f)) != LAMD_OK) return rc;
  hipLaunchKernelGGL(k_dedupe_insert_count, dim3(blocks_for(n)), dim3(256), 0, ctx->stream, n, c.d_key, c.keylen, c.keystride, root->hash_seed,
                     (const u32 *)f.row_ent, ctx->kd_table.as<u32>(), (u32)(f.m - 1), ctx->kd_rep.as<u32>(), f.plan, ctx->kd_uniq.as<u32>(), ctx->kd_count.as<u32>());
  launch_classify<true>(ctx, c, f);
  if (c.time_it) HIPCHK(ctx, hipEventRecord(ctx->ev[1], ctx->stream));
  if (ctx->early_cold) {
    hipLaunchKernelGGL(k_partition_cold, dim3(blocks_for(n)), dim3(256), 0, ctx->stream, n, ctx->kd_rep.as<const u32>(), ctx->kd_newent.as<const u32>(), f.plan,
                       f.listcold);
    if ((rc = launch_cold(ctx, c, f.listcold, f.plan, f.fin)) != LAMD_OK) return rc;
    *cold_started = true;
  }
  const bool on7 = f.thr[0] != NO_TABLES, on10 = f.thr[1] != NO_TABLES;
  if (on7 || on10) {
    const kc_shape_args A7 = shape_args(ctx->hk[0], on7 ? f.cap[0] : 0, kc->pool7), A10 = shape_args(ctx->hk[1], on10 ? f.cap[1] : 0, kc->pool10);
    const unsigned kb7 = on7 ? blocks_for(f.cap[0]) : 0u, kb10 = on10 ? blocks_for(f.cap[1]) : 0u;
    hipLaunchKernelGGL(k_keys_bases_both, dim3(kb7 + kb10), dim3(256), 0, ctx->stream, (const u32 *)f.plan, kb7, A7, A10, c.d_key, c.keylen, c.keystride);
    const publish_args P = {c.d_key, c.keylen, c.keystride, (u32)ctx->lane_id, f.seq ? f.seq : 1u, root->hash_seed, kc->ents.as<cache_ent>(), kc->index.as<u32>(),
                            kc->index_mask, (int)f.use_cache};
    if (root->kc_tree) {
      const unsigned tb7 = on7 ? (unsigned)((f.cap[0] + 64 * KC_TREE_KPL7 - 1) / (64 * KC_TREE_KPL7)) : 0u;
      const unsigned tb10 = on10 ? (unsigned)((f.cap[1] + 64 * KC_TREE_KPL10 - 1) / (64 * KC_TREE_KPL10)) : 0u;
      hipLaunchKernelGGL(k_kc_tree_both, dim3(tb7 + tb10), dim3(64), 0, ctx->stream, (const u32 *)f.plan, tb7, A7, A10, P);
    } else {
      const unsigned fb7 = on7 ? blocks_for(f.cap[0] * kc_nsub(7)) : 0u, fb10 = on10 ? blocks_for(f.cap[1] * kc_nsub(10)) : 0u;
      hipLaunchKernelGGL(k_kc_finish_both, dim3(fb7 + fb10), dim3(256), 0, ctx->stream, (const u32 *)f.plan, fb7, A7, A10, P);
    }
  }
  if ((rc = mark_published(ctx, root, f)) != LAMD_OK) return rc;
  auto part = *cold_started ? k_partition<true, true> : k_partition<true, false>;
  hipLaunchKernelGGL(part, dim3(blocks_for(n)), dim3(256), 0, ctx->stream, n, f.row_ent, ctx->kd_rep.as<const u32>(), (const u32 *)nullptr,
                     ctx->kd_newent.as<const u32>(), kc->ents.as<const cache_ent>(), f.plan, f.list7, f.list10, f.listcold, c.keyok_out, c.d_ok, c.d_sig, c.mode);
  return LAMD_OK;
}

static int front_end_legacy(lamd_ctx *ctx, lamd_ctx *root, const chunk_io &c, const front_args &f) {
  int rc;
  const size_t n = c.n;
  lamd_ctx::key_cache *kc = f.kc;
  HIPCHK(ctx, hipMemsetAsync(f.plan, 0, P_WORDS * 4, ctx->stream));
  HIPCHK(ctx, hipMemsetAsync(ctx->kd_table.p, 0, f.m * 4, ctx->stream));
  HIPCHK(ctx, hipMemsetAsync(ctx->kd_count.p, 0, n * 4, ctx->stream));
  if (f.use_cache) {
    if ((rc = launch_cache_lookup(ctx, root, c, f)) != LAMD_OK) return rc;
  } else {
    HIPCHK(ctx, hipMemsetAsync(f.row_ent, 0xFF, n * 4, ctx->stream));
    HIPCHK(ctx, hipMemsetAsync(f.cc, 0, C_WORDS * 4, ctx->stream));
  }
  hipLaunchKernelGGL(k_dedupe_insert, dim3(blocks_for(n)), dim3(256), 0, ctx->stream, n, c.d_key, c.keylen, c.keystride, root->hash_seed, (const u32 *)f.row_ent,
                     ctx->kd_table.as<u32>(), (u32)(f.m - 1), ctx->kd_rep.as<u32>());
  hipLaunchKernelGGL(k_dedupe_number, dim3(blocks_for(n)), dim3(256), 0, ctx->stream, n, ctx->kd_rep.as<const u32>(), ctx->kd_uid.as<u32>(), f.plan,
                     ctx->kd_uniq.as<u32>());
  hipLaunchKernelGGL(k_dedupe_map, dim3(blocks_for(n)), dim3(256), 0, ctx->stream, n, ctx->kd_rep.as<const u32>(), ctx->kd_uid.as<const u32>(), ctx->kd_count.as<u32>());
  launch_classify<false>(ctx, c, f);
  if (c.time_it) HIPCHK(ctx, hipEventRecord(ctx->ev[1], ctx->stream));
  for (int s = 0; s < 2; s++) {
    if (f.thr[s] == NO_TABLES) continue;
    const int which = s ? P_HK10 : P_HK7;
    const kc_shape_args A = shape_args(ctx->hk[s], f.cap[s], s ? kc->pool10 : kc->pool7);
    hipLaunchKernelGGL(k_keys, dim3(blocks_for(f.cap[s])), dim3(256), 0, ctx->stream, f.cap[s], c.d_key, c.keylen, c.keystride, A.hk_row, A.qwords, A.keyok,
                       (const u32 *)(f.plan + which));
    if (s) launch_keytables<10>(ctx->stream, f.plan, which, A);
    else launch_keytables<7>(ctx->stream, f.plan, which, A);
    hipLaunchKernelGGL(k_cache_publish, dim3(blocks_for(f.cap[s])), dim3(256), 0, ctx->stream, (const u32 *)f.plan, which, A.cap, A.hk_row, A.hk_ent, A.hk_slot,
                       A.keyok, c.d_key, c.keylen, c.keystride, s ? 10u : 7u, (u32)ctx->lane_id, f.seq ? f.seq : 1u, root->hash_seed, kc->ents.as<cache_ent>(),
                       kc->index.as<u32>(), kc->index_mask, (int)f.use_cache);
  }
  if ((rc = mark_published(ctx, root, f)) != LAMD_OK) return rc;
  hipLaunchKernelGGL((k_partition<false>), dim3(blocks_for(n)), dim3(256), 0, ctx->stream, n, f.row_ent, ctx->kd_rep.as<const u32>(), ctx->kd_uid.as<const u32>(),
                     ctx->kd_newent.as<const u32>(), kc->ents.as<const cache_ent>(), f.plan, f.list7, f.list10, f.listcold, c.keyok_out, c.d_ok, c.d_sig, c.mode);
  return LAMD_OK;
}

static int group_lists(lamd_ctx *ctx, size_t n, size_t ent_words, keyed_lists *k) {
  int rc;
  if (ctx->g_cnt.cap < ent_words * 4) {
    if ((rc = ensure(ctx, &ctx->g_cnt, ent_words * 4)) != LAMD_OK) return rc;
    HIPCHK(ctx, hipMemsetAsync(ctx->g_cnt.p, 0, ctx->g_cnt.cap, ctx->stream));
  }
  if ((rc = ensure(ctx, &ctx->g_base, ent_words * 4)) != LAMD_OK) return rc;
  for (devbuf *b : {&ctx->g_rank, &ctx->g_touched, &ctx->g_list7, &ctx->g_list10})
    if ((rc = ensure(ctx, b, n * 4)) != LAMD_OK) return rc;
  hipLaunchKernelGGL(k_group_count, dim3(blocks_for(n)), dim3(256), 0, ctx->stream, k->plan, k->list7, k->list10, k->row_ent, ctx->g_cnt.as<u32>(),
                     ctx->g_rank.as<u32>(), ctx->g_touched.as<u32>());
  hipLaunchKernelGGL(k_group_alloc, dim3(blocks_for(n)), dim3(256), 0, ctx->stream, k->plan, ctx->g_touched.as<const u32>(), k->ents, ctx->g_cnt.as<u32>(),
                     ctx->g_base.as<u32>());
  hipLaunchKernelGGL(k_group_scatter, dim3(blocks_for(n)), dim3(256), 0, ctx->stream, (const u32 *)k->plan, k->list7, k->list10, k->row_ent,
                     ctx->g_base.as<const u32>(), ctx->g_rank.as<const u32>(), ctx->g_list7.as<u32>(), ctx->g_list10.as<u32>());
  k->list7 = ctx->g_list7.as<const u32>();
  k->list10 = ctx->g_list10.as<const u32>();
  return LAMD_OK;
}

static int ecmult_stage(lamd_ctx *ctx, lamd_ctx *root, const chunk_io &c, size_t ent_words, keyed_lists k) {
  int rc;
  const size_t n = c.n;
  if (ctx->group_rows && n >= 4096 && (rc = group_lists(ctx, n, ent_words, &k)) != LAMD_OK) return rc;
  if (c.time_it) HIPCHK(ctx, hipEventRecord(ctx->ev[2], ctx->stream));
  HIPCHK(ctx, hipStreamWaitEvent(ctx->stream, ctx->ev_prep, 0));
  const bool chain = root->ecm_chain != 0 && n >= root->ecm_chain_min;
  if (chain && root->ecm_last >= 0 && root->ecm_last != ctx->lane_id) HIPCHK(ctx, hipStreamWaitEvent(ctx->stream, root->ev_ecm[root->ecm_last], 0));
  const bool time_kernel = c.time_it && ctx->kev_n < lamd_ctx::KEV;
  if (time_kernel) {
    hipEvent_t *pair = ctx->kev[ctx->kev_n];
    if (!pair[0]) {
      HIPCHK(ctx, hipEventCreate(&pair[0]));
      HIPCHK(ctx, hipEventCreate(&pair[1]));
    }
    HIPCHK(ctx, hipEventRecord(pair[0], ctx->stream));
  }
  const bool two_parts = chain && root->ecm_chain == 2 && ctx->stream_lo;
  if (two_parts) {
    HIPCHK(ctx, hipEventRecord(ctx->ev_lo_go, ctx->stream));
    HIPCHK(ctx, hipStreamWaitEvent(ctx->stream_lo, ctx->ev_lo_go, 0));
    launch_keyed<false>(ctx, ctx->stream_lo, (root->ecm_tail + KEYED_THREADS - 1) / KEYED_THREADS, c, k, 2, root->ecm_tail);
    HIPCHK(ctx, hipEventRecord(ctx->ev_lo_done, ctx->stream_lo));
  }
  if (ctx->pairs && !two_parts) {
    const unsigned resident = (unsigned)ctx->prop.multiProcessorCount * 3u * 4u, full = (unsigned)((n + PAIRS_THREADS - 1) / PAIRS_THREADS);
    const unsigned grid = full < resident ? full : resident;
    if ((rc = ensure(ctx, &ctx->pairs_ws, (size_t)PAIRS_SLOTS * PAIRS_WS_WORDS * 4 * grid * PAIRS_THREADS)) != LAMD_OK) return rc;
    hipLaunchKernelGGL((k_ecmult_keyed_pairs<3>), dim3(grid), dim3(PAIRS_THREADS), 0, ctx->stream, k.plan, k.list7, k.list10, (const prep_rec *)c.recs, k.row_ent, k.ents,
                       k.pool7, k.pool10, c.d_sig, c.mode, (const u32 *)ctx->gtable, k.fin, c.keyok_out, c.d_ok, ctx->pairs_ws.as<u32>());
  } else {
    launch_keyed<false>(ctx, ctx->stream, keyed_grid(n), c, k, two_parts ? 1 : 0, root->ecm_tail);
  }
  if (time_kernel) {
    HIPCHK(ctx, hipEventRecord(ctx->kev[ctx->kev_n][1], ctx->stream));
    ctx->kev_mode[ctx->kev_n++] = c.mode == MODE_SCHNORR ? 1 : 0;
  }
  if (chain) {
    HIPCHK(ctx, hipEventRecord(root->ev_ecm[ctx->lane_id], ctx->stream));
    root->ecm_last = ctx->lane_id;
  }
  if (two_parts) HIPCHK(ctx, hipStreamWaitEvent(ctx->stream, ctx->ev_lo_done, 0));
  launch_keyed<true>(ctx, ctx->stream, careful_grid(ctx, n), c, k);
  return LAMD_OK;
}

static void table_thresholds(const lamd_ctx *ctx, bool small, bool use_cache, bool latency_learn, u32 thr[2]) {
  u32 thr7 = ctx->keyed_mode > 0 ? 2u : (u32)(ctx->keyed_min_uses + 0.5), thr10 = (u32)(ctx->keyed_dense_uses + 0.5);
  if (ctx->keyed_teeth == 7) thr10 = NO_TABLES;
  if (ctx->keyed_teeth == 10) { thr10 = thr7; thr7 = NO_TABLES; }
  if (thr7 < 2) thr7 = 2;
  if (thr10 < 2) thr10 = 2;
  if (small) {
    thr7 = use_cache && ctx->small_fused && ctx->keyed_teeth != 10 ? 1u : NO_TABLES;
    if (ctx->keyed_teeth != 7) thr10 = (u32)(ctx->keyed_dense_uses + 0.5);
    if (latency_learn && ctx->keyed_teeth != 7) thr10 = 1u;
  }
  thr[0] = thr7;
  thr[1] = thr10;
}

static int chunk_partitioned(lamd_ctx *ctx, lamd_ctx *root, const chunk_io &c, bool use_cache, bool small, bool latency_learn) {
  int rc;
  const size_t n = c.n;
  front_args f = {};
  f.use_cache = use_cache;
  table_thresholds(ctx, small, use_cache, latency_learn, f.thr);
  for (int s = 0; s < 2; s++) f.cap[s] = f.thr[s] == NO_TABLES ? 1 : n / f.thr[s] + 1;
  lamd_ctx::key_cache *kc = f.kc = use_cache ? &root->cache_store : &ctx->cache_store;
  if (!use_cache && (rc = cache_alloc(ctx, kc, f.cap[0], f.cap[1], false)) != LAMD_OK) return rc;
  f.m = 4;
  while (f.m < 2 * n) f.m <<= 1;
  if ((rc = ensure(ctx, &ctx->kd_table, f.m * 4)) != LAMD_OK) return rc;
  for (devbuf *b : {&ctx->row_ent, &ctx->kd_rep, &ctx->kd_uid, &ctx->kd_uniq, &ctx->kd_count, &ctx->kd_newent, &ctx->list7, &ctx->list10,
                    &ctx->listcold})
    if ((rc = ensure(ctx, b, n * 4)) != LAMD_OK) return rc;
  for (int s = 0; s < 2; s++) {
    lamd_ctx::shape_ws &w = ctx->hk[s];
    for (devbuf *b : {&w.row, &w.ent, &w.slot})
      if ((rc = ensure(ctx, b, f.cap[s] * 4)) != LAMD_OK) return rc;
    if ((rc = ensure(ctx, &w.qwords, f.cap[s] * 64)) != LAMD_OK) return rc;
    if ((rc = ensure(ctx, &w.keyok, f.cap[s])) != LAMD_OK) return rc;
    if ((rc = ensure(ctx, &w.scratch, f.cap[s] * kc_scratch_words(s ? 10 : 7) * 4)) != LAMD_OK) return rc;
  }
  if ((rc = ensure(ctx, &ctx->plan, P_WORDS * 4)) != LAMD_OK) return rc;
  if (c.mode == MODE_SCHNORR && (rc = ensure(ctx, &ctx->kt_fin, n * (size_t)FIN_WORDS * 4)) != LAMD_OK) return rc;
  f.plan = ctx->plan.as<u32>();
  f.cc = kc->counters.as<u32>();
  f.row_ent = ctx->row_ent.as<u32>();
  f.list7 = ctx->list7.as<u32>();
  f.list10 = ctx->list10.as<u32>();
  f.listcold = ctx->listcold.as<u32>();
  f.fin = c.mode == MODE_SCHNORR ? ctx->kt_fin.as<u32>() : nullptr;
  if (use_cache) {
    f.vis = cache_visibility(root, ctx);
    f.seq = ++root->call_seq;
  }
  f.lf = {nullptr, 0, c.d_key, c.keylen, c.keystride, root->hash_seed, 0xFFFFFFFFu, 0xFFFFFFFFu};
  if (small && use_cache) {
    f.lf.budget7 = kc->cap7 / 2;
    f.lf.budget10 = kc->cap10 / 2;
    if (latency_learn && !ctx->learn_fps.empty()) {
      const size_t nf = ctx->learn_fps.size() < 4096 ? ctx->learn_fps.size() : 4096;
      if ((rc = ensure(ctx, &ctx->learn_dev, nf * 8)) != LAMD_OK) return rc;
      HIPCHK(ctx, hipMemcpyAsync(ctx->learn_dev.p, ctx->learn_fps.data(), nf * 8, hipMemcpyHostToDevice, ctx->stream));
      f.lf.fps = ctx->learn_dev.as<const u64>();
      f.lf.n = (u32)nf;
    }
  }
  bool cold_started = false;
  if ((rc = ctx->fused_front ? front_end_fused(ctx, root, c, f, &cold_started) : front_end_legacy(ctx, root, c, f)) != LAMD_OK) return rc;
  if (!cold_started && (rc = launch_cold(ctx, c, f.listcold, f.plan, f.fin)) != LAMD_OK) return rc;
  const keyed_lists k = {f.plan, f.list7, f.list10, f.row_ent, kc->ents.as<const cache_ent>(), kc->pool7.as<const u32>(), kc->pool10.as<const u32>(), f.fin};
  if ((rc = ecmult_stage(ctx, root, c, kc->cap_ent, k)) != LAMD_OK) return rc;
  HIPCHK(ctx, hipStreamWaitEvent(ctx->stream, ctx->ev_cold, 0));
  return finish_call(ctx, c, f.fin, f.plan, f.cc);
}

static int run_chunk(lamd_ctx *ctx, int mode, size_t n, const u8 *d_a, const u8 *d_sig, const u8 *d_key, int keylen,
                     size_t keystride, u8 *d_ok_caller, u8 *keyok_out, bool time_it) {
  int rc;
  lamd_ctx *root = ctx->root ? ctx->root : ctx;
  if ((rc = ensure(ctx, &ctx->recs, n * sizeof(prep_rec))) != LAMD_OK) return rc;
  if ((rc = ensure(ctx, &ctx->vbuf, n)) != LAMD_OK) return rc;
  const chunk_io c = {mode, n, d_sig, d_key, keylen, keystride, d_ok_caller, keyok_out, time_it, ctx->recs.as<prep_rec>(), ctx->vbuf.as<u8>()};
  if (time_it) HIPCHK(ctx, hipEventRecord(ctx->ev[0], ctx->stream));
  HIPCHK(ctx, hipEventRecord(ctx->ev_fork, ctx->stream));
  HIPCHK(ctx, hipStreamWaitEvent(ctx->stream2, ctx->ev_fork, 0));
  launch_prep(ctx, ctx->stream2, mode, n, d_a, d_sig, d_key, c.recs);
  HIPCHK(ctx, hipEventRecord(ctx->ev_prep, ctx->stream2));

  ctx->last_mode = mode;
  ctx->last_n = n;
  const bool use_cache = root->cache_mode != 0 && root->cache_store.shared;
  const bool small = n < ctx->keyed_min_rows && ctx->keyed_mode <= 0;
  const bool keyed = ctx->keyed_mode != 0 && n < 0x7FFFFFFFu && (use_cache || !small);
  ctx->last_keyed_call = keyed;
  if (!keyed) return chunk_direct(ctx, c);
  bool latency_learn = false;
  if (small && use_cache && ctx->small_fused) {
    const u32 dense_thr = ctx->last_small_n / 8 > 32 ? (u32)(ctx->last_small_n / 8) : 32u;
    const bool learn = ctx->force_learn || (ctx->last_small_fused && ctx->h_plan && ((volatile const u32 *)ctx->h_plan)[P_DENSE] >= dense_thr);
    latency_learn = ctx->force_learn;
    ctx->force_learn = false;
    ctx->last_small_fused = !learn;
    ctx->last_small_n = n;
    if (!learn) return chunk_small_cached(ctx, root, c);
  }
  return chunk_partitioned(ctx, root, c, use_cache, small, latency_learn);
}

static int cache_maybe_reset(lamd_ctx *root) {
  if (root->cache_mode == 0 || !root->cache_store.shared) return LAMD_OK;
  const lamd_ctx::key_cache &kc = root->cache_store;
  u32 hw[3] = {0, 0, 0};
  for (int i = 0; i <= MAX_LANES; i++) {
    const lamd_ctx *L = i < MAX_LANES ? root->lane[i] : root;
    if (!L || !L->h_plan) continue;
    for (int k = 0; k < 3; k++) {
      const u32 v = ((volatile const u32 *)L->h_plan)[P_WORDS + k];
      if (v > hw[k]) hw[k] = v;
    }
  }
  for (int k = 0; k < 3; k++) root->cache_hwm[k] = hw[k];
  if ((double)hw[0] > 0.9 * kc.cap_ent || (double)hw[1] > 0.9 * kc.cap7 || (double)hw[2] > 0.9 * kc.cap10) return cache_reset(root);
  return LAMD_OK;
}

static int run_device(lamd_ctx *ctx, int mode, size_t n, const u8 *d_a, const u8 *d_sig, const u8 *d_key, int keylen,
                      size_t keystride, u8 *d_ok, u8 *keyok_out = nullptr) {
  HIPCHK(ctx, hipSetDevice(ctx->device));
  if (!ctx->root) ctx->last_lane = nullptr;
  bool forked = false;
  size_t k = 0;
  for (size_t o = 0; o < n; o += ctx->chunk, k++) {
    const size_t m = n - o < ctx->chunk ? n - o : ctx->chunk;
    lamd_ctx *W = (k & 1) && ctx->peer ? ctx->peer : ctx;
    W->timing = ctx->timing;
    if (W != ctx && !forked) {
      HIPCHK(ctx, hipEventRecord(ctx->ev_lane, ctx->stream));
      HIPCHK(ctx, hipStreamWaitEvent(W->stream, ctx->ev_lane, 0));
      forked = true;
    }
    const int rc = run_chunk(W, mode, m, d_a + 32 * o, d_sig + 64 * o, d_key + keystride * o, keylen, keystride, d_ok + o,
                             keyok_out ? keyok_out + o : nullptr, ctx->timing && o + ctx->chunk >= n);
    ctx->last_chunk_lane = W;
    if (rc != LAMD_OK) {
      if (W != ctx) ctx->err = W->err;
      return rc;
    }
  }
  if (forked) {
    HIPCHK(ctx, hipEventRecord(ctx->peer->ev_join, ctx->peer->stream));
    HIPCHK(ctx, hipStreamWaitEvent(ctx->stream, ctx->peer->ev_join, 0));
  }
  return LAMD_OK;
}

extern "C" int lamd_verify_ecdsa_batch_device(lamd_ctx *ctx, size_t n, const void *d_hash32, const void *d_sig64,
                                              const void *d_pub, size_t publen, size_t pubstride, void *d_ok) {
  if (!ctx) return LAMD_ERR_ARG;
  if (n == 0) return LAMD_OK;
  if (!d_hash32 || !d_sig64 || !d_pub || !d_ok || (publen != 33 && publen != 65) || pubstride < publen) {
    ctx->err = "bad argument";
    return LAMD_ERR_ARG;
  }
  lamd_ctx *L;
  int rc = pick_lane(ctx, &L);
  if (rc != LAMD_OK) return rc;
  rc = run_device(L, MODE_ECDSA, n, (const u8 *)d_hash32, (const u8 *)d_sig64, (const u8 *)d_pub, (int)publen, pubstride, (u8 *)d_ok);
  if (rc != LAMD_OK && L != ctx) ctx->err = L->err;
  return rc;
}

extern "C" int lamd_verify_schnorr_batch_device(lamd_ctx *ctx, size_t n, const void *d_msg32, const void *d_xonly32,
                                                const void *d_sig64, void *d_ok) {
  if (!ctx) return LAMD_ERR_ARG;
  if (n == 0) return LAMD_OK;
  if (!d_msg32 || !d_xonly32 || !d_sig64 || !d_ok) {
    ctx->err = "bad argument";
    return LAMD_ERR_ARG;
  }
  lamd_ctx *L;
  int rc = pick_lane(ctx, &L);
  if (rc != LAMD_OK) return rc;
  rc = run_device(L, MODE_SCHNORR, n, (const u8 *)d_msg32, (const u8 *)d_sig64, (const u8 *)d_xonly32, 32, 32, (u8 *)d_ok);
  if (rc != LAMD_OK && L != ctx) ctx->err = L->err;
  return rc;
}

constexpr size_t SMALL_MAX = 4096;
constexpr size_t TXSIG_HOST_HASH_ROWS = 16;
constexpr size_t SMALL_OFF_SIG = SMALL_MAX * 32, SMALL_OFF_KEY = SMALL_OFF_SIG + SMALL_MAX * 64, SMALL_OFF_OUT = SMALL_OFF_KEY + SMALL_MAX * 65 + 64,
                 SMALL_OFF_SHAPES = SMALL_OFF_OUT + SMALL_MAX, SMALL_OFF_FLAG = SMALL_OFF_SHAPES + SMALL_MAX, SMALL_BYTES = SMALL_OFF_FLAG + 64;
constexpr size_t MISS_SLOTS = 65536, MISS_WAYS = 4;
static inline u64 *miss_bucket(std::vector<u64> &t, u64 fp) { return &t[((fp >> 1) % (MISS_SLOTS / MISS_WAYS)) * MISS_WAYS]; }
static inline bool miss_has(std::vector<u64> &t, u64 fp) {
  const u64 *b = miss_bucket(t, fp);
  return b[0] == fp || b[1] == fp || b[2] == fp || b[3] == fp;
}
static inline void miss_put(std::vector<u64> &t, u64 fp) {
  u64 *b = miss_bucket(t, fp);
  for (size_t w = 0; w < MISS_WAYS; w++)
    if (b[w] == fp) return;
  for (size_t w = 0; w < MISS_WAYS; w++)
    if (b[w] == 0) { b[w] = fp; return; }
  b[(fp >> 40) % MISS_WAYS] = fp;
}
static inline bool miss_take(std::vector<u64> &t, u64 fp) {
  u64 *b = miss_bucket(t, fp);
  for (size_t w = 0; w < MISS_WAYS; w++)
    if (b[w] == fp) { b[w] = 0; return true; }
  return false;
}
__host__ __device__ static inline u64 small_fingerprint(u64 seed, const u8 *key, int keylen) {
  u64 h = seed ^ 0x6D697373ull;
  for (int o = 0; o < keylen; o += 8) {
    u64 c = 0;
    for (int b = 0; b < 8 && o + b < keylen; b++) c |= (u64)key[o + b] << (8 * b);
    h = (h ^ c) * 0x9E3779B97F4A7C15ull;
    h ^= h >> 29;
  }
  return h | 1;
}
static void small_forget(lamd_ctx *ctx, lamd_ctx *dst, const u8 *key, size_t keystride, int keylen, size_t n) {
  dst->learn_fps.clear();
  for (size_t i = 0; i < n; i++) {
    if (i && memcmp(key + i * keystride, key + (i - 1) * keystride, keylen) == 0) continue;
    const u64 fp = small_fingerprint(ctx->hash_seed, key + i * keystride, keylen);
    if (miss_take(ctx->small_missed, fp)) dst->learn_fps.push_back(fp);
  }
}
static int run_small(lamd_ctx *ctx, int mode, size_t n, const u8 *a, const u8 *sig, const u8 *key, int keylen, size_t keystride, u8 *ok,
                     const u8 *d_a32 = nullptr, const u8 *d_gate = nullptr) {
  int rc;
  if (!ctx->h_small) {
    HIPCHK(ctx, hipHostMalloc((void **)&ctx->h_small, SMALL_BYTES, hipHostMallocMapped | hipHostMallocCoherent));
    memset(ctx->h_small, 0, SMALL_BYTES);
  }
  if ((rc = ensure(ctx, &ctx->slots, ((n + 63) & ~(size_t)63) * SLOT_WORDS * 4)) != LAMD_OK) return rc;
  if (!ctx->small_done.p) {
    if ((rc = ensure(ctx, &ctx->small_done, 64)) != LAMD_OK) return rc;
    HIPCHK(ctx, hipMemsetAsync(ctx->small_done.p, 0, 64, ctx->stream));
  }
  u8 *h = ctx->h_small;
  const bool have_cache = ctx->cache_mode != 0 && ctx->cache_store.shared;
  if (have_cache) {
    if (ctx->small_missed.empty()) ctx->small_missed.assign(MISS_SLOTS, 0);
    bool learn = false;
    for (size_t i = 0; i < n && !learn; i++) {
      if (i && memcmp(key + i * keystride, key + (i - 1) * keystride, keylen) == 0) continue;
      const u64 fp = small_fingerprint(ctx->hash_seed, key + i * keystride, keylen);
      learn = miss_has(ctx->small_missed, fp);
    }
    if (learn) {
      small_forget(ctx, ctx, key, keystride, keylen, n);
      return 1;
    }
  }
  if (!d_a32) memcpy(h, a, n * 32);
  memcpy(h + SMALL_OFF_SIG, sig, n * 64);
  if (keystride == (size_t)keylen) memcpy(h + SMALL_OFF_KEY, key, n * keylen);
  else
    for (size_t i = 0; i < n; i++) memcpy(h + SMALL_OFF_KEY + i * keylen, key + i * keystride, keylen);
  memset(h + SMALL_OFF_OUT, 0xEE, n);
  memset(h + SMALL_OFF_SHAPES, 0xEE, n);
  small_args A;
// ... 564 lines not shown
  if (!hash32 || !sig64 || !recid || !pub33 || !ok) {
    ctx->err = "bad argument";
    return LAMD_ERR_ARG;
  }
  HIPCHK(ctx, hipSetDevice(ctx->device));
  int rc;
  if ((rc = ensure(ctx, &ctx->in_a, n * 32)) != LAMD_OK) return rc;
  if ((rc = ensure(ctx, &ctx->in_b, n * 64)) != LAMD_OK) return rc;
  if ((rc = ensure(ctx, &ctx->in_c, n * 34)) != LAMD_OK) return rc;
  if ((rc = ensure(ctx, &ctx->out, n)) != LAMD_OK) return rc;
  u8 *d_recid = ctx->in_c.as<u8>(), *d_keys = d_recid + n;
  HIPCHK(ctx, hipMemcpyAsync(ctx->in_a.p, hash32, n * 32, hipMemcpyHostToDevice, ctx->stream));
  HIPCHK(ctx, hipMemcpyAsync(ctx->in_b.p, sig64, n * 64, hipMemcpyHostToDevice, ctx->stream));
  HIPCHK(ctx, hipMemcpyAsync(d_recid, recid, n, hipMemcpyHostToDevice, ctx->stream));
  rc = recover_device(ctx, n, ctx->in_a.as<const u8>(), ctx->in_b.as<const u8>(), d_recid, d_keys, ctx->out.as<u8>());
  if (rc != LAMD_OK) return rc;
  HIPCHK(ctx, hipMemcpyAsync(pub33, d_keys, n * 33, hipMemcpyDeviceToHost, ctx->stream));
  HIPCHK(ctx, hipMemcpyAsync(ok, ctx->out.p, n, hipMemcpyDeviceToHost, ctx->stream));
  return lamd_synchronize(ctx);
}

extern "C" int lamd_grind_htlc_tx_fee(lamd_ctx *ctx, const uint8_t *preimage, size_t preimage_len, const uint8_t *outputs,
                                      size_t outputs_len, uint64_t input_sat, uint64_t weight, uint32_t min_feerate,
                                      uint32_t max_feerate, const uint8_t sig64[64], uint8_t sighash_type, int has_witness_script,
                                      const uint8_t pubkey33[33], uint32_t *feerate, uint64_t *fee) {
  if (!ctx) return LAMD_ERR_ARG;
  if (!preimage || !outputs || !sig64 || !pubkey33 || !feerate || !fee || preimage_len < 40 + 4 || outputs_len < 9 ||
      outputs_len > (size_t)GRIND_MAX_OUTPUTS || weight == 0 || weight > ((uint64_t)1 << 31)) {
    ctx->err = "bad argument";
    return LAMD_ERR_ARG;
  }
  if (!(sighash_type == 1 || (sighash_type == 0x83 && has_witness_script))) return 0;
  if (max_feerate < min_feerate) return 0;
  const size_t ncand = (size_t)max_feerate - min_feerate + 1;
  if (ncand > ((size_t)1 << 30)) {
    ctx->err = "feerate range too large";
    return LAMD_ERR_ARG;
  }
  HIPCHK(ctx, hipSetDevice(ctx->device));
  const size_t lead = ((preimage_len - 40) / 64) * 64, tail_len = preimage_len - lead;
  const size_t o_out = (preimage_len + 15) & ~(size_t)15, o_sig = (o_out + outputs_len + 15) & ~(size_t)15, o_key = o_sig + 64,
               o_setup = o_key + 48, o_best = o_setup + ((sizeof(grind_setup) + 15) & ~(size_t)15), total = o_best + 16;
  int rc;
  if ((rc = ensure(ctx, &ctx->g_msgs, total)) != LAMD_OK) return rc;
  if ((rc = ensure(ctx, &ctx->slots, (size_t)SLOT_WORDS * 4)) != LAMD_OK) return rc;
  std::vector<u8> stage(total, 0);
  memcpy(&stage[0], preimage, preimage_len);
  memcpy(&stage[o_out], outputs, outputs_len);
  memcpy(&stage[o_sig], sig64, 64);
  memcpy(&stage[o_key], pubkey33, 33);
  memset(&stage[o_best], 0xFF, 4);
  u8 *d = ctx->g_msgs.as<u8>();
  HIPCHK(ctx, hipMemcpyAsync(d, stage.data(), total, hipMemcpyHostToDevice, ctx->stream));
  hipLaunchKernelGGL(k_grind_setup, dim3(1), dim3(64), 0, ctx->stream, d + o_sig, d + o_key, d, (u32)(lead / 64), ctx->slots.as<u32>(),
                     (const u32 *)ctx->gtable, (grind_setup *)(d + o_setup));
  hipLaunchKernelGGL(k_grind, dim3(blocks_for(ncand)), dim3(256), 0, ctx->stream, (u32)ncand, min_feerate, weight, input_sat, d + lead,
                     (u32)tail_len, (u32)lead, d + o_out, (u32)outputs_len, (const grind_setup *)(d + o_setup), (const u32 *)ctx->gtable,
                     (u32 *)(d + o_best));
  HIPCHK(ctx, hipGetLastError());
  u32 best = 0xFFFFFFFFu;
  HIPCHK(ctx, hipMemcpyAsync(&best, d + o_best, 4, hipMemcpyDeviceToHost, ctx->stream));
  HIPCHK(ctx, hipStreamSynchronize(ctx->stream));
  if (best == 0xFFFFFFFFu) return 0;
  *feerate = min_feerate + best;
  *fee = (uint64_t)*feerate * weight / 1000;
  return 1;
}

static int gossip_device(lamd_ctx *ctx, size_t n, const u8 *d_msgs, const u64 *d_off, const u8 *d_ids, const u64 *d_rowbase, size_t rows,
                         int8_t *d_verdict, const u64 *d_len = nullptr) {
  int rc;
  if ((rc = ensure(ctx, &ctx->g_hash, rows * 32)) != LAMD_OK) return rc;
  if ((rc = ensure(ctx, &ctx->g_sig, rows * 64)) != LAMD_OK) return rc;
  if ((rc = ensure(ctx, &ctx->g_pub, rows * 33 + 16)) != LAMD_OK) return rc;
  if ((rc = ensure(ctx, &ctx->g_malformed, n)) != LAMD_OK) return rc;
  if ((rc = ensure(ctx, &ctx->g_ok, rows)) != LAMD_OK) return rc;
  if ((rc = ensure(ctx, &ctx->keyok_row, rows)) != LAMD_OK) return rc;
  hipLaunchKernelGGL(k_gossip_expand, dim3(blocks_for(n)), dim3(256), 0, ctx->stream, n, d_msgs, d_off, d_len, d_ids, d_rowbase, ctx->g_hash.as<u8>(),
                     ctx->g_sig.as<u8>(), ctx->g_pub.as<u8>(), ctx->g_malformed.as<u8>());
  HIPCHK(ctx, hipGetLastError());
  rc = run_device(ctx, MODE_ECDSA, rows, ctx->g_hash.as<const u8>(), ctx->g_sig.as<const u8>(), ctx->g_pub.as<const u8>(), 33, 33, ctx->g_ok.as<u8>(),
                  ctx->keyok_row.as<u8>());
  if (rc != LAMD_OK) return rc;
  hipLaunchKernelGGL(k_gossip_reduce, dim3(blocks_for(n)), dim3(256), 0, ctx->stream, n, d_msgs, d_off, d_rowbase, ctx->g_ok.as<const u8>(),
                     ctx->keyok_row.as<const u8>(), ctx->g_malformed.as<const u8>(), d_verdict);
  HIPCHK(ctx, hipGetLastError());
  return LAMD_OK;
}

extern "C" int lamd_sigcheck_gossip_batch_device(lamd_ctx *ctx, size_t n, const void *d_msgs, const void *d_off, const void *d_node_ids33,
                                                 const void *d_rowbase, size_t rows, void *d_verdict) {
  if (!ctx) return LAMD_ERR_ARG;
  if (n == 0) return LAMD_OK;
  if (!d_msgs || !d_off || !d_rowbase || !d_verdict || rows == 0) {
    ctx->err = "bad argument";
    return LAMD_ERR_ARG;
  }
  HIPCHK(ctx, hipSetDevice(ctx->device));
  lamd_ctx *L;
  int rc = pick_lane(ctx, &L);
  if (rc != LAMD_OK) return rc;
  rc = gossip_device(L, n, (const u8 *)d_msgs, (const u64 *)d_off, (const u8 *)d_node_ids33, (const u64 *)d_rowbase, rows, (int8_t *)d_verdict);
  if (rc != LAMD_OK && L != ctx) ctx->err = L->err;
  return rc;
}

extern "C" int lamd_sigcheck_gossip_spans_device(lamd_ctx *ctx, size_t n, const void *d_msgs, const void *d_start, const void *d_len,
                                                 const void *d_node_ids33, const void *d_rowbase, size_t rows, void *d_verdict) {
  if (!ctx) return LAMD_ERR_ARG;
  if (n == 0) return LAMD_OK;
  if (!d_msgs || !d_start || !d_len || !d_rowbase || !d_verdict || rows == 0) {
    ctx->err = "bad argument";
    return LAMD_ERR_ARG;
  }
  HIPCHK(ctx, hipSetDevice(ctx->device));
  lamd_ctx *L;
  int rc = pick_lane(ctx, &L);
  if (rc != LAMD_OK) return rc;
  rc = gossip_device(L, n, (const u8 *)d_msgs, (const u64 *)d_start, (const u8 *)d_node_ids33, (const u64 *)d_rowbase, rows, (int8_t *)d_verdict,
                     (const u64 *)d_len);
  if (rc != LAMD_OK && L != ctx) ctx->err = L->err;
  return rc;
}

static void store_count_verdicts(const int8_t *v, size_t n, lamd_store_summary *s) {
  for (size_t i = 0; i < n; i++) {
    switch (v[i]) {
      case LAMD_STORE_OK: s->ok++; break;
      case LAMD_STORE_SKIPPED_DELETED: s->skipped_deleted++; break;
      case LAMD_STORE_BAD_CHECKSUM: s->bad_checksum++; break;
      case LAMD_STORE_UNKNOWN_TYPE: s->unknown_type++; break;
      case LAMD_STORE_MALFORMED: s->malformed++; break;
      case LAMD_STORE_REDUNDANT: s->redundant++; break;
      case LAMD_STORE_NO_CHANNEL: s->no_channel++; break;
      default:
        if (v[i] >= 1 && v[i] <= 4) s->bad_signature[v[i] - 1]++;
    }
  }
  s->clean = s->end_reason == LAMD_STORE_END_EOF && s->ok + s->skipped_deleted == n;
}
extern "C" int lamd_gossip_store_frame(const uint8_t *store, size_t len, size_t cap, uint64_t *rec_off, size_t *n_records,
                                       lamd_store_summary *summary) {
  if (!store || !n_records || !summary || (cap && !rec_off)) return LAMD_ERR_ARG;
  *n_records = 0;
  if (!store_walk(store, len, summary, [&](size_t i, u64 off, const store_hdr &, u32) {
        if (i < cap) rec_off[i] = off;
      }))
    return LAMD_ERR_ARG;
  *n_records = (size_t)summary->records;
  return summary->records > cap ? LAMD_ERR_ARG : LAMD_OK;
}
struct store_job {
  lamd_ctx *L = nullptr;
  size_t n = 0, n_cann = 0;
  const u8 *img = nullptr;
  const u64 *d_recoff = nullptr;
  const u64 *d_keys = nullptr;
  const u32 *d_vals = nullptr;
  u32 bits = 0;
  const int8_t *d_verdict = nullptr;
  std::vector<u64> pack;
};
#define STCHK(call) do { hipError_t e_ = (call); if (e_ != hipSuccess) { L->err = std::string(#call) + ": " + hipGetErrorString(e_); return fail(LAMD_ERR_HIP); } } while (0)
static int store_audit_queue(lamd_ctx *ctx, const uint8_t *store, size_t len, const void *d_store, size_t cap, uint64_t *rec_off, size_t *n_records,
                             lamd_store_summary *summary, store_job *job) {
  *n_records = 0;
  std::vector<u64> start, mlen, rowbase;
  std::vector<u32> sel;
  size_t n_cann = 0;
  u64 rows = 0;
  if (!store_walk(store, len, summary, [&](size_t i, u64 off, const store_hdr &h, u32 type) {
        if (i < cap) rec_off[i] = off;
        const bool sig = type == STORE_T_CANN || type == STORE_T_NANN || type == STORE_T_CUPD;
        sel.push_back(sig ? (u32)start.size() : STORE_NONE);
        if (!sig) return;
        start.push_back(off + STORE_HDR);
        mlen.push_back(h.len);
        rowbase.push_back(rows);
        rows += type == STORE_T_CANN ? 4 : 1;
        n_cann += type == STORE_T_CANN;
      })) {
    ctx->err = "not a gossip_store of major version 0";
    return LAMD_ERR_ARG;
  }
  const size_t n = (size_t)summary->records, nsel = start.size();
  *n_records = n;
  if (n > cap) { ctx->err = "gossip_store audit: rec_off / verdict too small"; return LAMD_ERR_ARG; }
  if (n >= (size_t)STORE_NONE || rows >= (u64)STORE_NONE) { ctx->err = "gossip_store audit: too many records"; return LAMD_ERR_ARG; }
  summary->signatures = rows;
  if (n == 0) return LAMD_OK;
  rowbase.push_back(rows);
  HIPCHK(ctx, hipSetDevice(ctx->device));
  lamd_ctx *L;
  int rc = pick_lane(ctx, &L);
  if (rc != LAMD_OK) return rc;
  u32 bits = 1;
  while (((size_t)1 << bits) < 2 * n_cann) bits++;
  const size_t slots = ((size_t)1 << bits) + 1;
  std::vector<u64> &pack = job->pack;
  pack.assign(n + 3 * nsel + 1 + (n + 1) / 2, 0);
// ... 513 lines not shown
  if (n <= SMALL_MAX || !ctx->use_copy_stream) return queue_push(ctx, kind, n, a, sig, key, Q_KEYBYTES[kind]);
  const size_t w[3] = {32, 64, Q_KEYBYTES[kind]};
  const u8 *col[3] = {a, sig, key};
  for (int c = 0; c < 3; c++)
    if (!g_registered.covers(col[c], w[c] * n)) return queue_push(ctx, kind, n, a, sig, key, Q_KEYBYTES[kind]);
  u8 *da, *db, *dc;
  const int first = queue_take(ctx, kind, n, &da, &db, &dc);
  if (first < 0) return first;
  lamd_ctx::queue &q = ctx->qs[ctx->q_open].q[kind];
  q.foreign.push_back({q.n - n, n, a, sig, key});
  return first;
}
extern "C" int lamd_queue_ecdsa_batch_inplace(lamd_ctx *ctx, size_t n, const uint8_t *hash32, const uint8_t *sig64, const uint8_t *pubkey, size_t publen) {
  if (ctx && publen != 33 && publen != 65) {
    ctx->err = "bad key length";
    return LAMD_ERR_ARG;
  }
  return queue_push_inplace(ctx, publen == 33 ? Q_ECDSA33 : Q_ECDSA65, n, hash32, sig64, pubkey);
}
extern "C" int lamd_queue_schnorr_batch_inplace(lamd_ctx *ctx, size_t n, const uint8_t *msg32, const uint8_t *xonly32, const uint8_t *sig64) {
  return queue_push_inplace(ctx, Q_SCHNORR, n, msg32, sig64, xonly32);
}
extern "C" int lamd_host_register(lamd_ctx *ctx, void *p, size_t bytes) {
  if (!ctx || !p || !bytes) return LAMD_ERR_ARG;
  if (hipSetDevice(ctx->device) != hipSuccess || hipHostRegister(p, bytes, hipHostRegisterPortable) != hipSuccess) {
    (void)hipGetLastError();
    return LAMD_ERR_HIP;
  }
  g_registered.add(p, bytes);
  return LAMD_OK;
}
extern "C" int lamd_device_numa_node(int device) {
  char bdf[64] = {0};
  if (hipDeviceGetPCIBusId(bdf, (int)sizeof bdf, device) != hipSuccess) {
    (void)hipGetLastError();
    return -1;
  }
  for (char *c = bdf; *c; c++) *c = (char)tolower((unsigned char)*c);
  const std::string path = std::string("/sys/bus/pci/devices/") + bdf + "/numa_node";
  FILE *f = fopen(path.c_str(), "r");
  if (!f) return -1;
  int node = -1;
  if (fscanf(f, "%d", &node) != 1) node = -1;
  fclose(f);
  return node;
}
extern "C" int lamd_host_unregister(lamd_ctx *ctx, void *p) {
  if (!ctx || !p) return LAMD_ERR_ARG;
  g_registered.remove(p);
  if (hipSetDevice(ctx->device) != hipSuccess || hipHostUnregister(p) != hipSuccess) {
    (void)hipGetLastError();
    return LAMD_ERR_HIP;
  }
  return LAMD_OK;
}
static int flush_open(lamd_ctx *ctx);
extern "C" int lamd_flush(lamd_ctx *ctx) {
  if (!ctx) return LAMD_ERR_ARG;
  if (ctx->q_open < 0) {
    ctx->err = "flush: every staging set is in flight (collect a flush with poll/wait first)";
    return LAMD_ERR_STATE;
  }
  const int rc = flush_open(ctx);
  if (rc < 0 && ctx->q_open >= 0) {
    (void)hipDeviceSynchronize();
    (void)hipGetLastError();
    lamd_ctx::queue_set &qs = ctx->qs[ctx->q_open];
    for (int kind = 0; kind < Q_KINDS; kind++) {
      lamd_ctx::queue &q = qs.q[kind];
      q.tickets.clear();
      q.foreign.clear();
      q.n = 0;
      q.small_flush = false;
    }
    qs.rows = 0;
    ctx->last_flush_inplace_rows = 0;
  }
  return rc;
}
static int flush_open(lamd_ctx *ctx) {
  HIPCHK(ctx, hipSetDevice(ctx->device));
  lamd_ctx::queue_set &qs = ctx->qs[ctx->q_open];
  lamd_ctx *L;
  int rc = pick_lane(ctx, &L);
  if (rc != LAMD_OK) return rc;
  for (int kind = 0; kind < Q_KINDS; kind++) {
    lamd_ctx::queue &q = qs.q[kind];
    if (!q.n) continue;
    const size_t kb = Q_KEYBYTES[kind];
    q.small_flush = false;
    if (q.n <= SMALL_MAX && ctx->small_kernel && ctx->keyed_mode <= 0 && ctx->cache_mode != 0 && ctx->cache_store.shared) {
      if (ctx->small_missed.empty()) ctx->small_missed.assign(MISS_SLOTS, 0);
      bool learn = false;
      for (size_t i = 0; i < q.n && !learn; i++) {
        if (i && memcmp(q.h_c + i * kb, q.h_c + (i - 1) * kb, kb) == 0) continue;
        const u64 fp = small_fingerprint(ctx->hash_seed, q.h_c + i * kb, (int)kb);
        learn = miss_has(ctx->small_missed, fp);
      }
      if (learn) {
        L->force_learn = true;
        small_forget(ctx, L, q.h_c, kb, (int)kb, q.n);
      } else {
        if ((rc = ensure(L, &L->slots, ((q.n + 63) & ~(size_t)63) * SLOT_WORDS * 4)) != LAMD_OK) { ctx->err = L->err; return rc; }
        small_args A;
        memset(&A, 0, sizeof A);
        A.a32 = q.h_a; A.sig64 = q.h_b; A.key = q.h_c;
        A.keylen = (int)kb; A.mode = kind == Q_SCHNORR ? MODE_SCHNORR : MODE_ECDSA; A.n = (u32)q.n;
        A.seed = ctx->hash_seed;
        lamd_ctx::key_cache *kc = &ctx->cache_store;
        for (int l = 0; l <= MAX_LANES; l++)
          if (ctx->pub_pending[l] && hipEventQuery(ctx->ev_pub[l]) == hipSuccess) {
            ctx->vis_seq[l] = ctx->pub_seq[l];
            ctx->pub_pending[l] = false;
          }
        (void)hipGetLastError();
        for (int l = 0; l <= MAX_LANES; l++) A.vis.seq[l] = ctx->vis_seq[l];
        A.vis.seq[L->lane_id] = ctx->pub_seq[L->lane_id];
        A.index = kc->index.as<const u32>(); A.mask = kc->index_mask; A.ents = kc->ents.as<const cache_ent>();
        A.pool7 = kc->pool7.as<const u32>(); A.pool10 = kc->pool10.as<const u32>();
        A.gtable = (const u32 *)ctx->gtable;
        A.slots = L->slots.as<u32>();
        A.out = q.h_ok;
        A.shapes = q.h_ok + q.cap;
        hipLaunchKernelGGL(k_small_verify, dim3((unsigned)((q.n + 63) / 64)), dim3(512), 0, L->stream, A);
        HIPCHK(ctx, hipGetLastError());
        q.small_flush = true;
        continue;
      }
    }
    if ((rc = ensure(ctx, &q.d_blk, lamd_ctx::queue::blk_bytes(q.cap, kb) + 64)) != LAMD_OK) return rc;
    if ((rc = ensure(ctx, &q.d_ok, q.n)) != LAMD_OK) return rc;
    u8 *const qd_c = q.d_blk.as<u8>(), *const qd_b = qd_c + lamd_ctx::queue::key_bytes_padded(q.cap, kb), *const qd_a = qd_b + q.cap * 64;
    const bool split = q.n <= L->chunk;
    if (!q.foreign.empty()) {
      hipStream_t &csr = ctx->copy_streams[ctx->copy_turn++ % (unsigned)ctx->n_copy_streams];
      if (!csr) HIPCHK(ctx, hipStreamCreateWithFlags(&csr, hipStreamNonBlocking));
      hipStream_t cs = csr;
      auto column = [&](int col) -> hipError_t {
        const size_t w = col == 0 ? kb : col == 1 ? 64 : 32;
        u8 *const dst = col == 0 ? qd_c : col == 1 ? qd_b : qd_a;
        const u8 *const own = col == 0 ? q.h_c : col == 1 ? q.h_b : q.h_a;
        size_t at = 0;
        hipError_t e = hipSuccess;
        for (const auto &f : q.foreign) {
          if (f.row0 > at && e == hipSuccess) e = hipMemcpyAsync(dst + at * w, own + at * w, (f.row0 - at) * w, hipMemcpyHostToDevice, cs);
          if (e == hipSuccess) e = hipMemcpyAsync(dst + f.row0 * w, col == 0 ? f.c : col == 1 ? f.b : f.a, f.count * w, hipMemcpyHostToDevice, cs);
          at = f.row0 + f.count;
        }
        if (at < q.n && e == hipSuccess) e = hipMemcpyAsync(dst + at * w, own + at * w, (q.n - at) * w, hipMemcpyHostToDevice, cs);
        return e;
      };
      const int events = ctx->copy_events ? ctx->copy_events : (ctx->q_inflight >= 2 ? 1 : 3);
      HIPCHK(ctx, column(0));
      if (events > 1) {
        HIPCHK(ctx, hipEventRecord(q.ev_keys, cs));
        HIPCHK(ctx, hipStreamWaitEvent(L->stream, q.ev_keys, 0));
      }
      HIPCHK(ctx, column(1));
      if (events >= 3) {
        HIPCHK(ctx, hipEventRecord(q.ev_sigs, cs));
        L->sigs_pending = true;
        L->ev_sigs_wait = q.ev_sigs;
      }
      HIPCHK(ctx, column(2));
      HIPCHK(ctx, hipEventRecord(q.ev_all, cs));
      if (events == 1) HIPCHK(ctx, hipStreamWaitEvent(L->stream, q.ev_all, 0));
      if (events == 2) {
        L->sigs_pending = true;
        L->ev_sigs_wait = q.ev_all;
      }
      HIPCHK(ctx, hipStreamWaitEvent(L->stream2, q.ev_all, 0));
    } else if (split && ctx->use_copy_stream) {
      hipStream_t &csr = ctx->copy_streams[ctx->copy_turn++ % (unsigned)ctx->n_copy_streams];
      if (!csr) HIPCHK(ctx, hipStreamCreateWithFlags(&csr, hipStreamNonBlocking));
      hipStream_t cs = csr;
      const int events = ctx->copy_events ? ctx->copy_events : (ctx->q_inflight >= 2 ? 1 : 3);
      if (events == 1 && q.n == q.cap && ctx->copy_one) {
        HIPCHK(ctx, hipMemcpyAsync(qd_c, q.h_blk, lamd_ctx::queue::blk_bytes(q.cap, kb), hipMemcpyHostToDevice, cs));
        HIPCHK(ctx, hipEventRecord(q.ev_all, cs));
        HIPCHK(ctx, hipStreamWaitEvent(L->stream, q.ev_all, 0));
        HIPCHK(ctx, hipStreamWaitEvent(L->stream2, q.ev_all, 0));
      } else if (events == 1) {
        HIPCHK(ctx, hipMemcpyAsync(qd_c, q.h_c, q.n * kb, hipMemcpyHostToDevice, cs));
        HIPCHK(ctx, hipMemcpyAsync(qd_b, q.h_b, q.n * 64, hipMemcpyHostToDevice, cs));
        HIPCHK(ctx, hipMemcpyAsync(qd_a, q.h_a, q.n * 32, hipMemcpyHostToDevice, cs));
        HIPCHK(ctx, hipEventRecord(q.ev_all, cs));
        HIPCHK(ctx, hipStreamWaitEvent(L->stream, q.ev_all, 0));
        HIPCHK(ctx, hipStreamWaitEvent(L->stream2, q.ev_all, 0));
      } else {
      HIPCHK(ctx, hipMemcpyAsync(qd_c, q.h_c, q.n * kb, hipMemcpyHostToDevice, cs));
      HIPCHK(ctx, hipEventRecord(q.ev_keys, cs));
      HIPCHK(ctx, hipStreamWaitEvent(L->stream, q.ev_keys, 0));
      HIPCHK(ctx, hipMemcpyAsync(qd_b, q.h_b, q.n * 64, hipMemcpyHostToDevice, cs));
      if (events >= 3) {
        HIPCHK(ctx, hipEventRecord(q.ev_sigs, cs));
        L->sigs_pending = true;
        L->ev_sigs_wait = q.ev_sigs;
      }
      HIPCHK(ctx, hipMemcpyAsync(qd_a, q.h_a, q.n * 32, hipMemcpyHostToDevice, cs));
      HIPCHK(ctx, hipEventRecord(q.ev_all, cs));
      if (events < 3) {
        L->sigs_pending = true;
        L->ev_sigs_wait = q.ev_all;
      }
      HIPCHK(ctx, hipStreamWaitEvent(L->stream2, q.ev_all, 0));
      }
    } else if (split) {
      HIPCHK(ctx, hipEventRecord(L->ev_fork, L->stream));
      HIPCHK(ctx, hipStreamWaitEvent(L->stream2, L->ev_fork, 0));
      HIPCHK(ctx, hipMemcpyAsync(qd_c, q.h_c, q.n * kb, hipMemcpyHostToDevice, L->stream2));
      HIPCHK(ctx, hipEventRecord(L->ev_keys, L->stream2));
      HIPCHK(ctx, hipStreamWaitEvent(L->stream, L->ev_keys, 0));
      HIPCHK(ctx, hipMemcpyAsync(qd_b, q.h_b, q.n * 64, hipMemcpyHostToDevice, L->stream2));
      HIPCHK(ctx, hipEventRecord(L->ev_sigs, L->stream2));
      L->sigs_pending = true;
      L->ev_sigs_wait = L->ev_sigs;
      HIPCHK(ctx, hipMemcpyAsync(qd_a, q.h_a, q.n * 32, hipMemcpyHostToDevice, L->stream2));
    } else {
      HIPCHK(ctx, hipMemcpyAsync(qd_c, q.h_c, q.n * kb, hipMemcpyHostToDevice, L->stream));
      HIPCHK(ctx, hipMemcpyAsync(qd_a, q.h_a, q.n * 32, hipMemcpyHostToDevice, L->stream));
      HIPCHK(ctx, hipMemcpyAsync(qd_b, q.h_b, q.n * 64, hipMemcpyHostToDevice, L->stream));
    }
    rc = run_device(L, kind == Q_SCHNORR ? MODE_SCHNORR : MODE_ECDSA, q.n, (const u8 *)qd_a, (const u8 *)qd_b,
                    (const u8 *)qd_c, (int)kb, kb, q.d_ok.as<u8>());
    L->force_learn = false;
    if (rc != LAMD_OK) {
      if (L != ctx) ctx->err = L->err;
      return rc;
    }
    HIPCHK(ctx, hipMemcpyAsync(q.h_ok, q.d_ok.p, q.n, hipMemcpyDeviceToHost, L->stream));
  }
  HIPCHK(ctx, hipEventRecord(qs.done, L->stream));
  size_t inplace = 0;
  for (int kind = 0; kind < Q_KINDS; kind++)
    for (const auto &f : qs.q[kind].foreign) inplace += f.count;
  ctx->last_flush_inplace_rows = inplace;
  ctx->q_fifo[ctx->q_inflight++] = ctx->q_open;
  ctx->q_open = -1;
  for (int sidx = 0; sidx < QUEUE_SETS && ctx->q_open < 0; sidx++) {
    bool busy = false;
    for (int k = 0; k < ctx->q_inflight; k++) busy |= ctx->q_fifo[k] == sidx;
    if (!busy) ctx->q_open = sidx;
  }
  return LAMD_OK;
}

static int collect(lamd_ctx *ctx, uint8_t *ok, size_t cap, size_t *n) {
  const int sidx = ctx->q_fifo[0];
  lamd_ctx::queue_set &qs = ctx->qs[sidx];
  const size_t total = qs.rows;
  if (total > cap) {
    ctx->err = "result buffer too small";
    return LAMD_ERR_ARG;
  }
  for (int kind = 0; kind < Q_KINDS; kind++) {
    lamd_ctx::queue &q = qs.q[kind];
    for (const auto &sp : q.tickets) memcpy(ok + sp.ticket0, q.h_ok + sp.row0, sp.count);
    if (q.small_flush && !ctx->small_missed.empty()) {
      const size_t kb = Q_KEYBYTES[kind];
      const u8 *shapes = q.h_ok + q.cap;
      for (size_t i = 0; i < q.n; i++)
        if (shapes[i] == 255 && !(i && shapes[i - 1] == 255 && memcmp(q.h_c + i * kb, q.h_c + (i - 1) * kb, kb) == 0)) {
          const u64 fp = small_fingerprint(ctx->hash_seed, q.h_c + i * kb, (int)kb);
          miss_put(ctx->small_missed, fp);
        }
    }
    q.small_flush = false;
    q.tickets.clear();
    q.foreign.clear();
    q.n = 0;
  }
  qs.rows = 0;
  if (n) *n = total;
  for (int k = 1; k < ctx->q_inflight; k++) ctx->q_fifo[k - 1] = ctx->q_fifo[k];
  ctx->q_inflight--;
  if (ctx->q_open < 0) ctx->q_open = sidx;
  return 1;
}
extern "C" int lamd_poll(lamd_ctx *ctx, uint8_t *ok, size_t cap, size_t *n) {
  if (!ctx || !ok) return LAMD_ERR_ARG;
  if (!ctx->q_inflight) {
    ctx->err = "poll before flush";
    return LAMD_ERR_STATE;
  }
  const hipError_t e = hipEventQuery(ctx->qs[ctx->q_fifo[0]].done);
  if (e == hipErrorNotReady) return 0;
  HIPCHK(ctx, e);
  return collect(ctx, ok, cap, n);
}
extern "C" int lamd_wait(lamd_ctx *ctx, uint8_t *ok, size_t cap, size_t *n) {
  if (!ctx || !ok) return LAMD_ERR_ARG;
  if (!ctx->q_inflight) {
    ctx->err = "wait before flush";
    return LAMD_ERR_STATE;
  }
  HIPCHK(ctx, hipEventSynchronize(ctx->qs[ctx->q_fifo[0]].done));
  return collect(ctx, ok, cap, n);
}

constexpr int ST_LANES = 64;
constexpr int ST_WORDS = 512;
struct st_in { u32 a[8], b[8]; u8 hash[32], sig[64], pub33[33], pad[3]; };

LAMD_HD void selftest_lane(const st_in &in, const u32 *gtable, u32 *slot, u32 *o) {
  int k = 0;
  const fe a = fe_from_words(in.a), b = fe_from_words(in.b);
  u32 w[8];
  fe_to_words(w, fe_normalize(fe_mul(a, b))); for (int i = 0; i < 8; i++) o[k++] = w[i];
  fe_to_words(w, fe_normalize(fe_sqr(a))); for (int i = 0; i < 8; i++) o[k++] = w[i];
  fe_to_words(w, fe_normalize(fe_inv(a))); for (int i = 0; i < 8; i++) o[k++] = w[i];
  fe_to_words(w, fe_normalize(fe_sqrt_candidate(a))); for (int i = 0; i < 8; i++) o[k++] = w[i];
  fe_to_words(w, fe_normalize(fe_add(fe_neg(a, 1), fe_mul_int(b, 3)))); for (int i = 0; i < 8; i++) o[k++] = w[i];
  sc x, y;
  bool of;
  x = sc_from_words(in.a, &of); y = sc_from_words(in.b, &of);
// ... 423 lines not shown
```

### lightning_amd/engine.py

```python
import ctypes

import numpy as np

from . import _ffi

ERRORS = {0: "OK", -1: "no usable gfx950 device", -2: "HIP error", -3: "bad argument", -4: "out of memory", -5: "bad state"}


class LamdError(RuntimeError):
    pass


def _u8(a, shape_tail):
    a = np.ascontiguousarray(a, dtype=np.uint8)
    if a.ndim == 1:
        a = a.reshape(-1, shape_tail)
    if a.shape[1] != shape_tail:
        raise ValueError("expected rows of %d bytes, got %r" % (shape_tail, a.shape))
    return a


def _key_column(pub, layout):
    if layout is None:
        pub = np.ascontiguousarray(pub, dtype=np.uint8)
# ... 394 lines not shown
        n, publen = d_pub.shape
        self._after_torch()
        self._chk(_ffi.load_testgen().lamd_gen_ecdsa_device(self._ctx, n, seed, nkeys, group, publen, d_hash.data_ptr(), d_sig.data_ptr(), d_pub.data_ptr()))

    def gen_schnorr_device(self, seed, nkeys, d_msg, d_xonly, d_sig, group=0):
        n = d_msg.shape[0]
        self._after_torch()
        self._chk(_ffi.load_testgen().lamd_gen_schnorr_device(self._ctx, n, seed, nkeys, group, d_msg.data_ptr(), d_xonly.data_ptr(), d_sig.data_ptr()))

    def gen_gossip_device(self, seed, n_cann, n_cupd, n_nodes, d_msgs, d_ids):
        self._after_torch()
        self._chk(_ffi.load_testgen().lamd_gen_gossip_device(self._ctx, n_cann, n_cupd, seed, n_nodes, d_msgs.data_ptr(), d_ids.data_ptr()))

    def sigcheck_gossip_device(self, n, d_msgs, d_off, d_ids, d_rowbase, rows, d_verdict):
        self._after_torch()
        self._chk(self._lib.lamd_sigcheck_gossip_batch_device(self._ctx, n, d_msgs.data_ptr(), d_off.data_ptr(),
                                                              d_ids.data_ptr() if d_ids is not None else None, d_rowbase.data_ptr(), rows,
                                                              d_verdict.data_ptr()))

    def sigcheck_gossip_spans_device(self, n, d_msgs, d_start, d_len, d_ids, d_rowbase, rows, d_verdict):
        self._after_torch()
        self._chk(self._lib.lamd_sigcheck_gossip_spans_device(self._ctx, n, d_msgs.data_ptr(), d_start.data_ptr(), d_len.data_ptr(),
                                                              d_ids.data_ptr() if d_ids is not None else None, d_rowbase.data_ptr(), rows,
                                                              d_verdict.data_ptr()))

    def selftest(self, hash32, sig64, pub33):
        buf = ctypes.create_string_buffer(4096)
        rc = self._chk(self._lib.lamd_selftest(self._ctx, bytes(hash32), bytes(sig64), bytes(pub33), buf, 4096))
        return rc, buf.value.decode()

    def chain_debug(self, use_mul):
        buf = ctypes.create_string_buffer(8192)
        rc = self._chk(self._lib.lamd_chain_debug(self._ctx, int(use_mul), buf, 8192))
        return rc, buf.value.decode()

    def inv_debug(self):
        buf = ctypes.create_string_buffer(8192)
        rc = self._chk(self._lib.lamd_inv_debug(self._ctx, buf, 8192))
        return rc, buf.value.decode()

    def fuzz_field(self, lanes=16384, iters=64, seed=1):
        buf = ctypes.create_string_buffer(4096)
        ops = ctypes.c_uint64(0)
        rc = self._chk(self._lib.lamd_fuzz_field(self._ctx, lanes, iters, seed, ctypes.byref(ops), buf, 4096))
        return rc, ops.value, buf.value.decode()

    def synchronize(self):
        self._chk(self._lib.lamd_synchronize(self._ctx))

    @property
    def stream_ptr(self):
        return self._lib.lamd_stream(self._ctx)

    def set_timing(self, on=True):
        self._chk(self._lib.lamd_set_timing(self._ctx, int(on)))

    def set_ecmult_chain(self, on):
        self._chk(self._lib.lamd_set_ecmult_chain(self._ctx, int(on)))

    def stream_wait_results(self, stream_ptr):
        self._chk(self._lib.lamd_stream_wait_results(self._ctx, ctypes.c_void_p(stream_ptr)))

    def wait_event(self, event_ptr):
        self._chk(self._lib.lamd_wait_event(self._ctx, ctypes.c_void_p(event_ptr)))

    def results_mark(self, slot):
        self._chk(self._lib.lamd_results_mark(self._ctx, int(slot)))

    def results_mark_last(self, slot):
        self._chk(self._lib.lamd_results_mark_last(self._ctx, slot))

    def stream_wait_mark(self, slot, stream_ptr):
        self._chk(self._lib.lamd_stream_wait_mark(self._ctx, int(slot), ctypes.c_void_p(stream_ptr)))

    def wait_stream(self, stream_ptr):
        self._chk(self._lib.lamd_wait_stream(self._ctx, ctypes.c_void_p(stream_ptr)))

    def info(self, lane=None):
        inf = _ffi.LamdInfo()
        if lane is None:
            self._chk(self._lib.lamd_get_info(self._ctx, ctypes.byref(inf)))
        else:
            self._chk(self._lib.lamd_get_lane_info(self._ctx, int(lane), ctypes.byref(inf)))
        return dict(device=inf.device, compute_units=inf.compute_units, arch=inf.arch.decode(), gtable_bytes=inf.gtable_bytes,
                    last_kernel_ms=list(inf.last_kernel_ms), last_unique_keys=inf.last_unique_keys, last_hot_rows=inf.last_hot_rows, last_keyed=int(inf.last_keyed), last_mode=int(inf.last_mode), lanes=int(inf.lanes),
                    last_cache_hits=inf.last_cache_hits, last_cold_rows=inf.last_cold_rows, last_new_tables=inf.last_new_tables,
                    last_suspect_rows=inf.last_suspect_rows, cache_enabled=bool(inf.cache_enabled), cache_entries=inf.cache_entries,
                    cache_capacity=inf.cache_capacity, cache_resets=inf.cache_resets,
                    keyed_ecmult_ms_sum=list(inf.keyed_ecmult_ms_sum), keyed_ecmult_launches=list(inf.keyed_ecmult_launches), hw_queues_env=int(inf.hw_queues_env), queue_sets=int(inf.queue_sets),
                    last_flush_inplace_rows=int(inf.last_flush_inplace_rows))

    def set_chunk_rows(self, rows):
        self._chk(self._lib.lamd_set_chunk_rows(self._ctx, rows))

    def mul32_peak(self, waves_per_simd=3, min_ms=4.0, launches=5):
        r, ms, ck = ctypes.c_double(0), ctypes.c_double(0), ctypes.c_double(0)
        self._chk(self._lib.lamd_debug_mul32_peak(self._ctx, waves_per_simd, min_ms, launches, ctypes.byref(r), ctypes.byref(ms), ctypes.byref(ck)))
        return r.value, ms.value, ck.value

    def cache_clear(self):
        self._chk(self._lib.lamd_cache_clear(self._ctx))
```

Before: 251.1 million verifies/s.

## Add staged stream layout splitting front-end and ecmult onto shared streams

Adds a 'staged' stream layout. Lanes stop creating their own streams and borrow a small root-owned set: two front-end streams for prep and cold work, plus one or two ecmult streams. Event handoffs link the two stages. The staged layout is picked automatically when the hardware queue count cannot cover the per-lane streams; the aim is to avoid oversubscribing hardware queues while still overlapping prep with the keyed ecmult of another call. The cost is extra event record/wait traffic and stricter serialisation through the few shared ecmult streams.

New measurement: 256.0 million verifies/s, median of 5. +1.9%, better.

```diff
diff --git a/include/lightning_amd.h b/include/lightning_amd.h
--- a/include/lightning_amd.h
+++ b/include/lightning_amd.h
@@ -223,6 +223,7 @@
 } lamd_info;
 int lamd_get_info(lamd_ctx *ctx, lamd_info *info);
 int lamd_get_lane_info(lamd_ctx *ctx, int lane, lamd_info *info);
+int lamd_get_stream_layout(lamd_ctx *ctx, int *staged, int *streams);
 int lamd_set_timing(lamd_ctx *ctx, int enable);
 int lamd_cache_clear(lamd_ctx *ctx);
 int lamd_set_ecmult_chain(lamd_ctx *ctx, int enable);
diff --git a/lightning_amd/_build.py b/lightning_amd/_build.py
--- a/lightning_amd/_build.py
+++ b/lightning_amd/_build.py
@@ -15,7 +15,7 @@
 EXTRA = os.environ.get("LAMD_BUILD_FLAGS", "").split()
 
 ENGINE_TUS = [
-    ("lamd_engine.hip", _H("verify_core.h", "group.h", "fe.h", "fe_asm.inc", "fuzz.h", "scalar.h", "sha256.h", "lamd_common.h", "bolt12.h", "host_ranges.h", "key_column.h", "store_audit.h", "store_repair.h", "store_latest.h") +
+    ("lamd_engine.hip", _H("verify_core.h", "group.h", "fe.h", "fe_asm.inc", "fuzz.h", "scalar.h", "sha256.h", "lamd_common.h", "bolt12.h", "host_ranges.h", "key_column.h", "stream_layout.h", "store_audit.h", "store_repair.h", "store_latest.h") +
      _I("lightning_amd.h", "lightning_amd_debug.h"), HIPFLAGS + EXTRA),
     ("lamd_multi.cpp", _H("numa_cpus.h") + _I("lightning_amd.h", "lightning_amd_debug.h"), ["-O2", "-std=c++17", "-fPIC", "-pthread", "-Wall"]),
 ]
diff --git a/lightning_amd/_ffi.py b/lightning_amd/_ffi.py
--- a/lightning_amd/_ffi.py
+++ b/lightning_amd/_ffi.py
@@ -103,6 +103,7 @@
     "lamd_set_chunk_rows": (ctypes.c_int, [ctypes.c_void_p, c_sz]),
     "lamd_cache_clear": (ctypes.c_int, [ctypes.c_void_p]),
     "lamd_get_lane_info": (ctypes.c_int, [ctypes.c_void_p, ctypes.c_int, ctypes.POINTER(LamdInfo)]),
+    "lamd_get_stream_layout": (ctypes.c_int, [ctypes.c_void_p, ctypes.POINTER(ctypes.c_int), ctypes.POINTER(ctypes.c_int)]),
     "lamd_stream_wait_results": (ctypes.c_int, [ctypes.c_void_p, ctypes.c_void_p]),
     "lamd_wait_stream": (ctypes.c_int, [ctypes.c_void_p, ctypes.c_void_p]),
     "lamd_wait_event": (ctypes.c_int, [ctypes.c_void_p, ctypes.c_void_p]),
diff --git a/lightning_amd/csrc/lamd_engine.hip b/lightning_amd/csrc/lamd_engine.hip
--- a/lightning_amd/csrc/lamd_engine.hip
+++ b/lightning_amd/csrc/lamd_engine.hip
@@ -18,6 +18,7 @@
 #include "fuzz.h"
 #include "host_ranges.h"
 #include "key_column.h"
+#include "stream_layout.h"
 #include "store_audit.h"
 #include "store_repair.h"
 #include "store_latest.h"
@@ -1516,6 +1517,14 @@
   devbuf keyok_row;
   hipStream_t stream2 = nullptr;
   hipStream_t stream3 = nullptr;
+  hipStream_t stream_ec = nullptr;
+  hipEvent_t ev_front = nullptr;
+  hipEvent_t ev_tail = nullptr;
+  bool tail_loose = false;
+  bool borrows = false;
+  lamd_stream_layout layout = {LAMD_LAYOUT_LANES, 0, 0, 2};
+  hipStream_t fe_streams[LAMD_STAGED_FE] = {nullptr, nullptr}, ec_streams[2] = {nullptr, nullptr};
+  unsigned stage_call = 0;
   hipEvent_t ev_fork = nullptr, ev_prep = nullptr, ev_cold = nullptr, ev_keys = nullptr, ev_sigs = nullptr;
   bool sigs_pending = false;
   hipEvent_t ev_sigs_wait = nullptr;
@@ -1668,9 +1677,20 @@
 static int cache_maybe_reset(lamd_ctx *root);
 
 static int create_streams(lamd_ctx *ctx) {
-  HIPCHK(ctx, hipStreamCreateWithFlags(&ctx->stream, hipStreamNonBlocking));
-  HIPCHK(ctx, hipStreamCreateWithFlags(&ctx->stream2, hipStreamNonBlocking));
-  if (!getenv("LAMD_MERGE_SIDE") || atoi(getenv("LAMD_MERGE_SIDE")) != 0) ctx->stream3 = ctx->stream2;
+  const bool staged_root = !ctx->is_lane && ctx->layout.kind == LAMD_LAYOUT_STAGED;
+  ctx->borrows = ctx->is_lane && ctx->root->layout.kind == LAMD_LAYOUT_STAGED;
+  if (!ctx->borrows) HIPCHK(ctx, hipStreamCreateWithFlags(&ctx->stream, hipStreamNonBlocking));
+  if (staged_root) {
+    for (int i = 0; i < ctx->layout.ec_streams; i++) HIPCHK(ctx, hipStreamCreateWithFlags(&ctx->ec_streams[i], hipStreamNonBlocking));
+    for (int i = 0; i < ctx->layout.fe_streams; i++) HIPCHK(ctx, hipStreamCreateWithFlags(&ctx->fe_streams[i], hipStreamNonBlocking));
+    ctx->stream2 = ctx->fe_streams[ctx->layout.fe_streams - 1];
+  } else if (!ctx->borrows) {
+    HIPCHK(ctx, hipStreamCreateWithFlags(&ctx->stream2, hipStreamNonBlocking));
+  }
+  ctx->stream_ec = ctx->stream;
+  HIPCHK(ctx, hipEventCreateWithFlags(&ctx->ev_front, hipEventDisableTiming));
+  HIPCHK(ctx, hipEventCreateWithFlags(&ctx->ev_tail, hipEventDisableTiming));
+  if (staged_root || ctx->borrows || !getenv("LAMD_MERGE_SIDE") || atoi(getenv("LAMD_MERGE_SIDE")) != 0) ctx->stream3 = ctx->stream2;
   else HIPCHK(ctx, hipStreamCreateWithFlags(&ctx->stream3, hipStreamNonBlocking));
   HIPCHK(ctx, hipEventCreateWithFlags(&ctx->ev_cold, hipEventDisableTiming));
   HIPCHK(ctx, hipEventCreateWithFlags(&ctx->ev_keys, hipEventDisableTiming));
@@ -1741,7 +1761,29 @@
   for (int i = 0; i < count; i++) root->lane[i]->peer = root->lane[(i + 1) % count];
   return LAMD_OK;
 }
-static int pick_lane(lamd_ctx *root, lamd_ctx **out) {
+static int assign_streams(lamd_ctx *L, hipStream_t fe, hipStream_t ec) {
+  const bool ran_before = L->stream_ec != nullptr;
+  if (ran_before && L->tail_loose) HIPCHK(L, hipEventRecord(L->ev_tail, L->stream_ec));
+  L->stream = L->stream2 = L->stream3 = fe;
+  L->stream_ec = ec;
+  if (ran_before) HIPCHK(L, hipStreamWaitEvent(L->stream, L->ev_tail, 0));
+  L->tail_loose = true;
+  return LAMD_OK;
+}
+static int mark_tail(lamd_ctx *ctx) {
+  if (!ctx->borrows || ctx->stream_ec == ctx->stream) return LAMD_OK;
+  HIPCHK(ctx, hipEventRecord(ctx->ev_tail, ctx->stream_ec));
+  ctx->tail_loose = false;
+  return LAMD_OK;
+}
+static int front_done(lamd_ctx *ctx) {
+  if (ctx->stream_ec == ctx->stream) return LAMD_OK;
+  HIPCHK(ctx, hipEventRecord(ctx->ev_front, ctx->stream));
+  HIPCHK(ctx, hipStreamWaitEvent(ctx->stream_ec, ctx->ev_front, 0));
+  return LAMD_OK;
+}
+
+static int pick_lane(lamd_ctx *root, lamd_ctx **out, bool split = false) {
   *out = root;
   const int rcc = cache_maybe_reset(root);
   if (rcc != LAMD_OK) return rcc;
@@ -1750,6 +1792,12 @@
   root->next_lane = (root->next_lane + 1) % root->nlanes;
   root->last_lane = L;
   L->timing = root->timing;
+  if (L->borrows) {
+    const unsigned k = root->stage_call++;
+    hipStream_t fe = root->fe_streams[layout_fe_of_call(root->layout, k)];
+    const int rc = assign_streams(L, fe, split ? root->ec_streams[layout_ec_of_call(root->layout, k)] : fe);
+    if (rc != LAMD_OK) { root->err = L->err; return rc; }
+  }
   HIPCHK(root, hipEventRecord(root->ev_lane, root->stream));
   HIPCHK(root, hipStreamWaitEvent(L->stream, root->ev_lane, 0));
   *out = L;
@@ -1797,6 +1845,9 @@
   if (const char *w = getenv("LAMD_SMALL_KERNEL")) ctx->small_kernel = atoi(w) != 0;
   if (const char *w = getenv("LAMD_CACHE_KEYS")) ctx->cache_keys = (size_t)atoll(w) < 64 ? 64 : (size_t)atoll(w);
   if (const char *w = getenv("LAMD_CACHE_KEYS10")) ctx->cache_keys10 = (size_t)atoll(w) < 16 ? 16 : (size_t)atoll(w);
+  const char *lanes = getenv("LAMD_LANES");
+  const int nl = lanes ? atoi(lanes) : 6;
+  ctx->layout = stream_layout(hw_queues_from_env(), nl > MAX_LANES ? MAX_LANES : nl, parse_layout_knob(getenv("LAMD_STREAM_LAYOUT")));
   int rc = create_streams(ctx);
   if (rc != LAMD_OK) return rc;
   std::vector<u32> bases(GTABLE_WINDOWS * 16);
@@ -1849,8 +1900,6 @@
     if ((rc = cache_reset(ctx)) != LAMD_OK) return rc;
     ctx->cache_resets = 0;
   }
-  const char *lanes = getenv("LAMD_LANES");
-  const int nl = lanes ? atoi(lanes) : 6;
   if (nl > 1) {
     rc = make_lanes(ctx, nl > MAX_LANES ? MAX_LANES : nl);
     if (rc != LAMD_OK) return rc;
@@ -1861,10 +1910,15 @@
 extern "C" void lamd_shutdown(lamd_ctx *ctx) {
   if (!ctx) return;
   (void)hipSetDevice(ctx->device);
+  for (hipStream_t st : {ctx->fe_streams[0], ctx->fe_streams[1], ctx->ec_streams[0], ctx->ec_streams[1]})
+    if (st) (void)hipStreamSynchronize(st);
+  if (ctx->borrows) ctx->stream = ctx->stream2 = ctx->stream3 = ctx->stream_ec = nullptr;
   for (auto &L : ctx->lane) {
     if (L) lamd_shutdown(L);
     L = nullptr;
   }
+  for (hipStream_t *st : {&ctx->fe_streams[0], &ctx->fe_streams[1]})
+    if (*st && (ctx->stream2 == *st || ctx->stream3 == *st)) ctx->stream2 = ctx->stream3 = nullptr;
   for (hipStream_t cs : ctx->copy_streams)
     if (cs) (void)hipStreamSynchronize(cs);
   if (ctx->stream) (void)hipStreamSynchronize(ctx->stream);
@@ -1925,6 +1979,10 @@
     if (e) (void)hipEventDestroy(e);
   if (ctx->ev_lane) (void)hipEventDestroy(ctx->ev_lane);
   if (ctx->ev_join) (void)hipEventDestroy(ctx->ev_join);
+  for (hipEvent_t e : {ctx->ev_front, ctx->ev_tail})
+    if (e) (void)hipEventDestroy(e);
+  for (hipStream_t st : {ctx->fe_streams[0], ctx->fe_streams[1], ctx->ec_streams[0], ctx->ec_streams[1]})
+    if (st) (void)hipStreamDestroy(st);
   for (auto &e : ctx->ev)
     if (e) (void)hipEventDestroy(e);
   for (auto &pair : ctx->kev)
@@ -1946,7 +2004,10 @@
     const int rc = lamd_synchronize(L);
     if (rc != LAMD_OK) { ctx->err = L->err; return rc; }
   }
-  HIPCHK(ctx, hipStreamSynchronize(ctx->stream));
+  for (hipStream_t st : {ctx->fe_streams[0], ctx->fe_streams[1], ctx->ec_streams[0], ctx->ec_streams[1]})
+    if (st) HIPCHK(ctx, hipStreamSynchronize(st));
+  if (ctx->stream) HIPCHK(ctx, hipStreamSynchronize(ctx->stream));
+  if (ctx->stream_ec && ctx->stream_ec != ctx->stream) HIPCHK(ctx, hipStreamSynchronize(ctx->stream_ec));
   if (ctx->timing && ctx->ev_recorded) {
     for (int i = 0; i < 4; i++) {
       float ms = 0;
@@ -1970,8 +2031,8 @@
   if (!ctx) return LAMD_ERR_ARG;
   for (int i = 0; i <= MAX_LANES; i++) {
     lamd_ctx *L = i < MAX_LANES ? ctx->lane[i] : ctx;
-    if (!L) continue;
-    HIPCHK(ctx, hipEventRecord(L->ev_join, L->stream));
+    if (!L || !L->stream_ec) continue;
+    HIPCHK(ctx, hipEventRecord(L->ev_join, L->stream_ec));
     HIPCHK(ctx, hipStreamWaitEvent((hipStream_t)stream, L->ev_join, 0));
   }
   return LAMD_OK;
@@ -1989,7 +2050,7 @@
     hipEvent_t &e = ctx->ev_mark[slot][i];
     if (!L) continue;
     if (!e) HIPCHK(ctx, hipEventCreateWithFlags(&e, hipEventDisableTiming));
-    HIPCHK(ctx, hipEventRecord(e, L->stream));
+    HIPCHK(ctx, hipEventRecord(e, L->stream_ec ? L->stream_ec : ctx->stream));
   }
   ctx->mark_set[slot] = true;
   ctx->mark_only[slot] = -1;
@@ -2004,7 +2065,7 @@
     if (ctx->lane[i] && ctx->lane[i] == ctx->last_lane) { idx = i; L = ctx->lane[i]; }
   hipEvent_t &e = ctx->ev_mark[slot][idx];
   if (!e) HIPCHK(ctx, hipEventCreateWithFlags(&e, hipEventDisableTiming));
-  HIPCHK(ctx, hipEventRecord(e, L->stream));
+  HIPCHK(ctx, hipEventRecord(e, L->stream_ec ? L->stream_ec : ctx->stream));
   ctx->mark_set[slot] = true;
   ctx->mark_only[slot] = idx;
   return LAMD_OK;
@@ -2059,6 +2120,14 @@
   if (!ctx) return LAMD_ERR_ARG;
   ctx->ecm_chain = enable != 0;
   ctx->ecm_last = -1;
+  return LAMD_OK;
+}
+
+extern "C" int lamd_get_stream_layout(lamd_ctx *ctx, int *staged, int *streams) {
+  if (!ctx) return LAMD_ERR_ARG;
+  const lamd_ctx *root = ctx->root ? ctx->root : ctx;
+  if (staged) *staged = root->layout.kind == LAMD_LAYOUT_STAGED;
+  if (streams) *streams = root->layout.streams;
   return LAMD_OK;
 }
 
@@ -2244,27 +2313,30 @@
 }
 
 static int finish_call(lamd_ctx *ctx, const chunk_io &c, u32 *fin, const u32 *plan, const u32 *cc) {
-  if (c.time_it) HIPCHK(ctx, hipEventRecord(ctx->ev[3], ctx->stream));
+  hipStream_t se = ctx->stream_ec;
+  if (c.time_it) HIPCHK(ctx, hipEventRecord(ctx->ev[3], se));
   if (c.mode == MODE_SCHNORR) {
     const unsigned blocks = blocks_for(final_threads(ctx, c.n));
-    if (fin) hipLaunchKernelGGL(k_schnorr_final_fin, dim3(blocks), dim3(256), 0, ctx->stream, c.n, fin, c.d_ok);
-    else hipLaunchKernelGGL(k_schnorr_final, dim3(blocks), dim3(256), 0, ctx->stream, c.n, ctx->slots.as<u32>(), c.d_ok);
-  }
-  HIPCHK(ctx, hipMemcpyAsync(c.d_ok_caller, c.d_ok, c.n, hipMemcpyDeviceToDevice, ctx->stream));
-  if (plan) HIPCHK(ctx, hipMemcpyAsync(ctx->h_plan, plan, P_WORDS * 4, hipMemcpyDeviceToHost, ctx->stream));
-  if (cc) HIPCHK(ctx, hipMemcpyAsync(ctx->h_plan + P_WORDS, cc, C_WORDS * 4, hipMemcpyDeviceToHost, ctx->stream));
+    if (fin) hipLaunchKernelGGL(k_schnorr_final_fin, dim3(blocks), dim3(256), 0, se, c.n, fin, c.d_ok);
+    else hipLaunchKernelGGL(k_schnorr_final, dim3(blocks), dim3(256), 0, se, c.n, ctx->slots.as<u32>(), c.d_ok);
+  }
+  HIPCHK(ctx, hipMemcpyAsync(c.d_ok_caller, c.d_ok, c.n, hipMemcpyDeviceToDevice, se));
+  if (plan) HIPCHK(ctx, hipMemcpyAsync(ctx->h_plan, plan, P_WORDS * 4, hipMemcpyDeviceToHost, se));
+  if (cc) HIPCHK(ctx, hipMemcpyAsync(ctx->h_plan + P_WORDS, cc, C_WORDS * 4, hipMemcpyDeviceToHost, se));
   if (c.time_it) {
-    HIPCHK(ctx, hipEventRecord(ctx->ev[4], ctx->stream));
+    HIPCHK(ctx, hipEventRecord(ctx->ev[4], se));
     ctx->ev_recorded = true;
   }
   HIPCHK(ctx, hipGetLastError());
-  return LAMD_OK;
+  return mark_tail(ctx);
 }
 
 static int chunk_direct(lamd_ctx *ctx, const chunk_io &c) {
   if (c.time_it) HIPCHK(ctx, hipEventRecord(ctx->ev[1], ctx->stream));
+  int rc2;
   const int rc = launch_direct(ctx, ctx->stream, c.mode, c.n, nullptr, nullptr, c.recs, c.d_sig, c.d_key, c.keylen, c.keystride, nullptr, c.keyok_out, c.d_ok, c.time_it);
   if (rc != LAMD_OK) return rc;
+  if ((rc2 = front_done(ctx)) != LAMD_OK) return rc2;
   return finish_call(ctx, c, nullptr, nullptr, nullptr);
 }
 
@@ -2287,10 +2359,11 @@
   if (c.time_it) HIPCHK(ctx, hipEventRecord(ctx->ev[1], ctx->stream));
   if ((rc = launch_cold(ctx, c, ctx->listcold.as<const u32>(), plan, k.fin)) != LAMD_OK) return rc;
   if (c.time_it) HIPCHK(ctx, hipEventRecord(ctx->ev[2], ctx->stream));
-  HIPCHK(ctx, hipStreamWaitEvent(ctx->stream, ctx->ev_prep, 0));
-  launch_keyed<false>(ctx, ctx->stream, keyed_grid(n), c, k);
-  launch_keyed<true>(ctx, ctx->stream, careful_grid(ctx, n), c, k);
-  HIPCHK(ctx, hipStreamWaitEvent(ctx->stream, ctx->ev_cold, 0));
+  if ((rc = front_done(ctx)) != LAMD_OK) return rc;
+  HIPCHK(ctx, hipStreamWaitEvent(ctx->stream_ec, ctx->ev_prep, 0));
+  launch_keyed<false>(ctx, ctx->stream_ec, keyed_grid(n), c, k);
+  launch_keyed<true>(ctx, ctx->stream_ec, careful_grid(ctx, n), c, k);
+  HIPCHK(ctx, hipStreamWaitEvent(ctx->stream_ec, ctx->ev_cold, 0));
   return finish_call(ctx, c, k.fin, plan, nullptr);
 }
 
@@ -2448,9 +2521,11 @@
   const size_t n = c.n;
   if (ctx->group_rows && n >= 4096 && (rc = group_lists(ctx, n, ent_words, &k)) != LAMD_OK) return rc;
   if (c.time_it) HIPCHK(ctx, hipEventRecord(ctx->ev[2], ctx->stream));
-  HIPCHK(ctx, hipStreamWaitEvent(ctx->stream, ctx->ev_prep, 0));
+  if ((rc = front_done(ctx)) != LAMD_OK) return rc;
+  hipStream_t se = ctx->stream_ec;
+  HIPCHK(ctx, hipStreamWaitEvent(se, ctx->ev_prep, 0));
   const bool chain = root->ecm_chain != 0 && n >= root->ecm_chain_min;
-  if (chain && root->ecm_last >= 0 && root->ecm_last != ctx->lane_id) HIPCHK(ctx, hipStreamWaitEvent(ctx->stream, root->ev_ecm[root->ecm_last], 0));
+  if (chain && root->ecm_last >= 0 && root->ecm_last != ctx->lane_id) HIPCHK(ctx, hipStreamWaitEvent(se, root->ev_ecm[root->ecm_last], 0));
   const bool time_kernel = c.time_it && ctx->kev_n < lamd_ctx::KEV;
   if (time_kernel) {
     hipEvent_t *pair = ctx->kev[ctx->kev_n];
@@ -2458,11 +2533,11 @@
       HIPCHK(ctx, hipEventCreate(&pair[0]));
       HIPCHK(ctx, hipEventCreate(&pair[1]));
     }
-    HIPCHK(ctx, hipEventRecord(pair[0], ctx->stream));
+    HIPCHK(ctx, hipEventRecord(pair[0], se));
   }
   const bool two_parts = chain && root->ecm_chain == 2 && ctx->stream_lo;
   if (two_parts) {
-    HIPCHK(ctx, hipEventRecord(ctx->ev_lo_go, ctx->stream));
+    HIPCHK(ctx, hipEventRecord(ctx->ev_lo_go, se));
     HIPCHK(ctx, hipStreamWaitEvent(ctx->stream_lo, ctx->ev_lo_go, 0));
     launch_keyed<false>(ctx, ctx->stream_lo, (root->ecm_tail + KEYED_THREADS - 1) / KEYED_THREADS, c, k, 2, root->ecm_tail);
     HIPCHK(ctx, hipEventRecord(ctx->ev_lo_done, ctx->stream_lo));
@@ -2471,21 +2546,21 @@
     const unsigned resident = (unsigned)ctx->prop.multiProcessorCount * 3u * 4u, full = (unsigned)((n + PAIRS_THREADS - 1) / PAIRS_THREADS);
     const unsigned grid = full < resident ? full : resident;
     if ((rc = ensure(ctx, &ctx->pairs_ws, (size_t)PAIRS_SLOTS * PAIRS_WS_WORDS * 4 * grid * PAIRS_THREADS)) != LAMD_OK) return rc;
-    hipLaunchKernelGGL((k_ecmult_keyed_pairs<3>), dim3(grid), dim3(PAIRS_THREADS), 0, ctx->stream, k.plan, k.list7, k.list10, (const prep_rec *)c.recs, k.row_ent, k.ents,
+    hipLaunchKernelGGL((k_ecmult_keyed_pairs<3>), dim3(grid), dim3(PAIRS_THREADS), 0, se, k.plan, k.list7, k.list10, (const prep_rec *)c.recs, k.row_ent, k.ents,
                        k.pool7, k.pool10, c.d_sig, c.mode, (const u32 *)ctx->gtable, k.fin, c.keyok_out, c.d_ok, ctx->pairs_ws.as<u32>());
   } else {
-    launch_keyed<false>(ctx, ctx->stream, keyed_grid(n), c, k, two_parts ? 1 : 0, root->ecm_tail);
+    launch_keyed<false>(ctx, se, keyed_grid(n), c, k, two_parts ? 1 : 0, root->ecm_tail);
   }
   if (time_kernel) {
-    HIPCHK(ctx, hipEventRecord(ctx->kev[ctx->kev_n][1], ctx->stream));
+    HIPCHK(ctx, hipEventRecord(ctx->kev[ctx->kev_n][1], se));
     ctx->kev_mode[ctx->kev_n++] = c.mode == MODE_SCHNORR ? 1 : 0;
   }
   if (chain) {
-    HIPCHK(ctx, hipEventRecord(root->ev_ecm[ctx->lane_id], ctx->stream));
+    HIPCHK(ctx, hipEventRecord(root->ev_ecm[ctx->lane_id], se));
     root->ecm_last = ctx->lane_id;
   }
-  if (two_parts) HIPCHK(ctx, hipStreamWaitEvent(ctx->stream, ctx->ev_lo_done, 0));
-  launch_keyed<true>(ctx, ctx->stream, careful_grid(ctx, n), c, k);
+  if (two_parts) HIPCHK(ctx, hipStreamWaitEvent(se, ctx->ev_lo_done, 0));
+  launch_keyed<true>(ctx, se, careful_grid(ctx, n), c, k);
   return LAMD_OK;
 }
 
@@ -2557,7 +2632,7 @@
   if (!cold_started && (rc = launch_cold(ctx, c, f.listcold, f.plan, f.fin)) != LAMD_OK) return rc;
   const keyed_lists k = {f.plan, f.list7, f.list10, f.row_ent, kc->ents.as<const cache_ent>(), kc->pool7.as<const u32>(), kc->pool10.as<const u32>(), f.fin};
   if ((rc = ecmult_stage(ctx, root, c, kc->cap_ent, k)) != LAMD_OK) return rc;
-  HIPCHK(ctx, hipStreamWaitEvent(ctx->stream, ctx->ev_cold, 0));
+  HIPCHK(ctx, hipStreamWaitEvent(ctx->stream_ec, ctx->ev_cold, 0));
   return finish_call(ctx, c, f.fin, f.plan, f.cc);
 }
 
@@ -2565,6 +2640,7 @@
                      size_t keystride, u8 *d_ok_caller, u8 *keyok_out, bool time_it) {
   int rc;
   lamd_ctx *root = ctx->root ? ctx->root : ctx;
+  if (ctx->stream_ec != ctx->stream && !ctx->tail_loose) HIPCHK(ctx, hipStreamWaitEvent(ctx->stream, ctx->ev_tail, 0));
   if ((rc = ensure(ctx, &ctx->recs, n * sizeof(prep_rec))) != LAMD_OK) return rc;
   if ((rc = ensure(ctx, &ctx->vbuf, n)) != LAMD_OK) return rc;
   const chunk_io c = {mode, n, d_sig, d_key, keylen, keystride, d_ok_caller, keyok_out, time_it, ctx->recs.as<prep_rec>(), ctx->vbuf.as<u8>()};
@@ -2621,6 +2697,10 @@
     const size_t m = n - o < ctx->chunk ? n - o : ctx->chunk;
     lamd_ctx *W = (k & 1) && ctx->peer ? ctx->peer : ctx;
     W->timing = ctx->timing;
+    if (W != ctx && !forked && W->borrows) {
+      const int rcs = assign_streams(W, ctx->stream, ctx->stream_ec);
+      if (rcs != LAMD_OK) { ctx->err = W->err; return rcs; }
+    }
     if (W != ctx && !forked) {
       HIPCHK(ctx, hipEventRecord(ctx->ev_lane, ctx->stream));
       HIPCHK(ctx, hipStreamWaitEvent(W->stream, ctx->ev_lane, 0));
@@ -2635,8 +2715,8 @@
     }
   }
   if (forked) {
-    HIPCHK(ctx, hipEventRecord(ctx->peer->ev_join, ctx->peer->stream));
-    HIPCHK(ctx, hipStreamWaitEvent(ctx->stream, ctx->peer->ev_join, 0));
+    HIPCHK(ctx, hipEventRecord(ctx->peer->ev_join, ctx->peer->stream_ec));
+    HIPCHK(ctx, hipStreamWaitEvent(ctx->stream_ec, ctx->peer->ev_join, 0));
   }
   return LAMD_OK;
 }
@@ -2650,7 +2730,7 @@
     return LAMD_ERR_ARG;
   }
   lamd_ctx *L;
-  int rc = pick_lane(ctx, &L);
+  int rc = pick_lane(ctx, &L, true);
   if (rc != LAMD_OK) return rc;
   rc = run_device(L, MODE_ECDSA, n, (const u8 *)d_hash32, (const u8 *)d_sig64, (const u8 *)d_pub, (int)publen, pubstride, (u8 *)d_ok);
   if (rc != LAMD_OK && L != ctx) ctx->err = L->err;
@@ -2666,7 +2746,7 @@
     return LAMD_ERR_ARG;
   }
   lamd_ctx *L;
-  int rc = pick_lane(ctx, &L);
+  int rc = pick_lane(ctx, &L, true);
   if (rc != LAMD_OK) return rc;
   rc = run_device(L, MODE_SCHNORR, n, (const u8 *)d_msg32, (const u8 *)d_sig64, (const u8 *)d_xonly32, 32, 32, (u8 *)d_ok);
   if (rc != LAMD_OK && L != ctx) ctx->err = L->err;
@@ -3397,10 +3477,10 @@
   rc = run_device(ctx, MODE_ECDSA, rows, ctx->g_hash.as<const u8>(), ctx->g_sig.as<const u8>(), ctx->g_pub.as<const u8>(), 33, 33, ctx->g_ok.as<u8>(),
                   ctx->keyok_row.as<u8>());
   if (rc != LAMD_OK) return rc;
-  hipLaunchKernelGGL(k_gossip_reduce, dim3(blocks_for(n)), dim3(256), 0, ctx->stream, n, d_msgs, d_off, d_rowbase, ctx->g_ok.as<const u8>(),
+  hipLaunchKernelGGL(k_gossip_reduce, dim3(blocks_for(n)), dim3(256), 0, ctx->stream_ec, n, d_msgs, d_off, d_rowbase, ctx->g_ok.as<const u8>(),
                      ctx->keyok_row.as<const u8>(), ctx->g_malformed.as<const u8>(), d_verdict);
   HIPCHK(ctx, hipGetLastError());
-  return LAMD_OK;
+  return mark_tail(ctx);
 }
 
 extern "C" int lamd_sigcheck_gossip_batch_device(lamd_ctx *ctx, size_t n, const void *d_msgs, const void *d_off, const void *d_node_ids33,
@@ -3413,7 +3493,7 @@
   }
   HIPCHK(ctx, hipSetDevice(ctx->device));
   lamd_ctx *L;
-  int rc = pick_lane(ctx, &L);
+  int rc = pick_lane(ctx, &L, true);
   if (rc != LAMD_OK) return rc;
   rc = gossip_device(L, n, (const u8 *)d_msgs, (const u64 *)d_off, (const u8 *)d_node_ids33, (const u64 *)d_rowbase, rows, (int8_t *)d_verdict);
   if (rc != LAMD_OK && L != ctx) ctx->err = L->err;
@@ -3430,7 +3510,7 @@
   }
   HIPCHK(ctx, hipSetDevice(ctx->device));
   lamd_ctx *L;
-  int rc = pick_lane(ctx, &L);
+  int rc = pick_lane(ctx, &L, true);
   if (rc != LAMD_OK) return rc;
   rc = gossip_device(L, n, (const u8 *)d_msgs, (const u64 *)d_start, (const u8 *)d_node_ids33, (const u64 *)d_rowbase, rows, (int8_t *)d_verdict,
                      (const u64 *)d_len);
@@ -4110,8 +4190,9 @@
   HIPCHK(ctx, hipSetDevice(ctx->device));
   lamd_ctx::queue_set &qs = ctx->qs[ctx->q_open];
   lamd_ctx *L;
-  int rc = pick_lane(ctx, &L);
+  int rc = pick_lane(ctx, &L, true);
   if (rc != LAMD_OK) return rc;
+  bool general = false;
   for (int kind = 0; kind < Q_KINDS; kind++) {
     lamd_ctx::queue &q = qs.q[kind];
     if (!q.n) continue;
@@ -4249,6 +4330,7 @@
       HIPCHK(ctx, hipMemcpyAsync(qd_a, q.h_a, q.n * 32, hipMemcpyHostToDevice, L->stream));
       HIPCHK(ctx, hipMemcpyAsync(qd_b, q.h_b, q.n * 64, hipMemcpyHostToDevice, L->stream));
     }
+    general = true;
     rc = run_device(L, kind == Q_SCHNORR ? MODE_SCHNORR : MODE_ECDSA, q.n, (const u8 *)qd_a, (const u8 *)qd_b,
                     (const u8 *)qd_c, (int)kb, kb, q.d_ok.as<u8>());
     L->force_learn = false;
@@ -4256,9 +4338,11 @@
       if (L != ctx) ctx->err = L->err;
       return rc;
     }
-    HIPCHK(ctx, hipMemcpyAsync(q.h_ok, q.d_ok.p, q.n, hipMemcpyDeviceToHost, L->stream));
-  }
-  HIPCHK(ctx, hipEventRecord(qs.done, L->stream));
+    HIPCHK(ctx, hipMemcpyAsync(q.h_ok, q.d_ok.p, q.n, hipMemcpyDeviceToHost, L->stream_ec));
+  }
+  if (!general && L->borrows) L->stream_ec = L->stream;
+  if ((rc = front_done(L)) != LAMD_OK || (rc = mark_tail(L)) != LAMD_OK) { ctx->err = L->err; return rc; }
+  HIPCHK(ctx, hipEventRecord(qs.done, L->stream_ec));
   size_t inplace = 0;
   for (int kind = 0; kind < Q_KINDS; kind++)
     for (const auto &f : qs.q[kind].foreign) inplace += f.count;
diff --git a/lightning_amd/csrc/stream_layout.h b/lightning_amd/csrc/stream_layout.h
--- /dev/null
+++ b/lightning_amd/csrc/stream_layout.h
@@ -0,0 +1,49 @@
+#pragma once
+
+enum lamd_layout_kind { LAMD_LAYOUT_LANES = 0, LAMD_LAYOUT_STAGED = 1 };
+enum lamd_layout_knob { LAMD_LAYOUT_KNOB_AUTO = 0, LAMD_LAYOUT_KNOB_LANES = 1, LAMD_LAYOUT_KNOB_STAGED = 2 };
+
+struct lamd_stream_layout {
+  int kind;
+  int fe_streams;
+  int ec_streams;
+  int streams;
+  int queues;
+};
+
+constexpr int LAMD_STAGED_FE = 2;
+
+static inline int layout_queues(int hw_queues_env) { return hw_queues_env > 0 ? hw_queues_env : 4; }
+
+static inline int layout_lanes_streams(int lanes) { return lanes > 1 ? 2 * lanes : 2; }
+static inline int layout_lanes_queues(int lanes) { return lanes > 1 ? lanes + 1 : 2; }
+
+static inline int parse_layout_knob(const char *v) {
+  if (!v || !*v) return LAMD_LAYOUT_KNOB_AUTO;
+  const char *a = "lanes", *b = "staged";
+  const char *p = v;
+  while (*a && *p == *a) { a++; p++; }
+  if (!*a && !*p) return LAMD_LAYOUT_KNOB_LANES;
+  p = v;
+  while (*b && *p == *b) { b++; p++; }
+  if (!*b && !*p) return LAMD_LAYOUT_KNOB_STAGED;
+  return LAMD_LAYOUT_KNOB_AUTO;
+}
+
+static inline lamd_stream_layout stream_layout(int hw_queues_env, int lanes, int knob) {
+  const int queues = layout_queues(hw_queues_env);
+  lamd_stream_layout l = {LAMD_LAYOUT_LANES, 0, 0, layout_lanes_streams(lanes), layout_lanes_queues(lanes)};
+  if (lanes <= 1) return l;
+  const bool staged = knob == LAMD_LAYOUT_KNOB_STAGED || (knob == LAMD_LAYOUT_KNOB_AUTO && queues - 1 < l.queues);
+  if (!staged) return l;
+  l.kind = LAMD_LAYOUT_STAGED;
+  l.fe_streams = LAMD_STAGED_FE;
+  l.ec_streams = queues >= 6 ? 2 : 1;
+  l.streams = l.queues = l.fe_streams + l.ec_streams;
+  return l;
+}
+
+static inline int layout_fe_of_call(const lamd_stream_layout &l, unsigned call) { return l.fe_streams ? (int)(call % (unsigned)l.fe_streams) : -1; }
+static inline int layout_ec_of_call(const lamd_stream_layout &l, unsigned call) { return l.ec_streams ? (int)(call % (unsigned)l.ec_streams) : -1; }
+
+static inline const char *layout_name(int kind) { return kind == LAMD_LAYOUT_STAGED ? "staged" : "lanes"; }
diff --git a/lightning_amd/engine.py b/lightning_amd/engine.py
--- a/lightning_amd/engine.py
+++ b/lightning_amd/engine.py
@@ -500,13 +500,15 @@
             self._chk(self._lib.lamd_get_info(self._ctx, ctypes.byref(inf)))
         else:
             self._chk(self._lib.lamd_get_lane_info(self._ctx, int(lane), ctypes.byref(inf)))
+        staged, streams = ctypes.c_int(0), ctypes.c_int(0)
+        self._chk(self._lib.lamd_get_stream_layout(self._ctx, ctypes.byref(staged), ctypes.byref(streams)))
         return dict(device=inf.device, compute_units=inf.compute_units, arch=inf.arch.decode(), gtable_bytes=inf.gtable_bytes,
                     last_kernel_ms=list(inf.last_kernel_ms), last_unique_keys=inf.last_unique_keys, last_hot_rows=inf.last_hot_rows, last_keyed=int(inf.last_keyed), last_mode=int(inf.last_mode), lanes=int(inf.lanes),
                     last_cache_hits=inf.last_cache_hits, last_cold_rows=inf.last_cold_rows, last_new_tables=inf.last_new_tables,
                     last_suspect_rows=inf.last_suspect_rows, cache_enabled=bool(inf.cache_enabled), cache_entries=inf.cache_entries,
                     cache_capacity=inf.cache_capacity, cache_resets=inf.cache_resets,
                     keyed_ecmult_ms_sum=list(inf.keyed_ecmult_ms_sum), keyed_ecmult_launches=list(inf.keyed_ecmult_launches), hw_queues_env=int(inf.hw_queues_env), queue_sets=int(inf.queue_sets),
-                    last_flush_inplace_rows=int(inf.last_flush_inplace_rows))
+                    last_flush_inplace_rows=int(inf.last_flush_inplace_rows), stream_layout="staged" if staged.value else "lanes", stream_layout_streams=int(streams.value))
 
     def set_chunk_rows(self, rows):
         self._chk(self._lib.lamd_set_chunk_rows(self._ctx, rows))
```
